# IDEA-Research/MP-Former

Hardware: AMD Instinct MI355X
Metric: training images/sec COCO-instance R50 1024x1024 (higher is better)
Workload: dtype bf16 (backbone, decoder) + f32 (pixel decoder, losses), as the reference's AMP; 1 GPU; COCO-instance R50, 100 queries, 80 classes, 1024x1024: full train step = R50 backbone + MSDeformAttn pixel decoder (6 layers) + MP masked decoder (9 layers, NUM_DN 1) + Hungarian matching + 60 losses + backward + grad all-reduce + clip + AdamW; head_only_workload=False, global_batch=2, per_gpu_batch=2, parallelism=dp1, msda_offsets=init, full=False, autograd_threads=backward on the launch thread, miopen_find_db=shipped

## Files before the change

include/mpformer_hip.h:

```cpp
#ifndef MPFORMER_HIP_H
#define MPFORMER_HIP_H

#include <stddef.h>
#include <stdint.h>

#ifdef __cplusplus
extern "C" {
#endif

enum { MPF_F32 = 0, MPF_F64 = 1, MPF_BF16 = 2, MPF_U8 = 3, MPF_BITS = 4  };

enum {
    MPF_OK = 0,
    MPF_E_DTYPE = -1,
    MPF_E_SHAPE = -2,
    MPF_E_NULL = -3,
    MPF_E_TOO_LARGE = -4
};

int mpf_abi_version(void);
const char* mpf_last_error(void);


int mpf_msda_forward(const void* value, const int64_t* spatial_shapes,
// ... 331 lines not shown
                      int Cout, int transposed, void* stream);
int mpf_gemm3_conv3x3_wgrad(const float* dy, const float* x, float* c_part, float* csum_dy, int n_img, int H, int W, int Cin, int Cout,
                            int rows_per_split, void* stream);

int mpf_gemm3_tn_ex(const void* a, int a_dtype, int64_t lda, const void* b_planes, const float* bias, const float* c_in, int64_t ldcin,
                    void* c, int c_dtype, int64_t ldc, int M, int N, int K, int relu, void* stream);
int mpf_gemm3_nt_ex(const void* a, int a_dtype, int64_t lda, const void* b, int b_dtype, int64_t ldb, float* c_part, float* csum_a,
                    int R, int Mdim, int Ndim, int rows_per_split, void* stream);

typedef struct MpfSplitItem {
    const float* src;
    void* dst;
    int64_t rows, cols, transpose, dst_ld, plane_stride, first_block;
} MpfSplitItem;

int mpf_gemm3_split_grouped(const MpfSplitItem* items_device, int n_items, int64_t total_blocks, void* stream);

typedef struct MpfOptItem {
    float* param;
    const float* grad;
    float* exp_avg;
    float* exp_avg_sq;
    int64_t numel, first_block;
    float lr, weight_decay, bc1, bc2_sqrt;
} MpfOptItem;

int mpf_clip_adamw_step(const MpfOptItem* items_device, int n_items, int64_t total_blocks, float max_norm, double beta1,
                        double beta2, double eps, float* partial, float* norm_clip, void* stream);

int mpf_transpose_f32(const float* in, int64_t in_batch_stride, float* out, int64_t out_batch_stride, int B, int R, int C,
                      void* stream);

int mpf_gemm3_nt_reduce(const float* c_part, int64_t c_numel, const float* s_part, int64_t s_numel, int nsplit,
                        float* c_out, float* s_out, void* stream);
int mpf_gemm3_nt_reduce_levels(const float* c_part, int64_t c_numel, const float* s_part, int64_t s_numel, int nsplit,
                               const int64_t* level_of_split, int n_levels, float* c_out, float* lvl_out, float* s_out, void* stream);

int mpf_tall_gemm_bf16(const void* a, int64_t lda, const void* b, int64_t ldb, const void* bias, void* c, int64_t ldc, int M, int N,
                       int K, void* stream);
size_t mpf_gemm_nt_bf16_workspace_bytes(int R, int Mdim, int Ndim, int rows_per_split);
int mpf_gemm_nt_bf16(const void* a, int64_t lda, const void* b, int64_t ldb, void* c_out, void* csum_out, int R, int Mdim,
                     int Ndim, int rows_per_split, void* workspace, size_t workspace_bytes, void* stream);

int mpf_small_gemm_bf16_blocked(const void* a, int64_t a_rs, int64_t a_ks, int a_blk, int64_t a_bs, const void* gate, const void* b,
                                int64_t b_rs, int64_t b_ks, const void* bias, const void* c_in, int64_t ldcin, void* c, int64_t ldc,
                                int c_blk, int64_t c_bs, void* rowsum_a, int I, int J, int Kc, int relu, void* stream);

int mpf_class_loss_forward(const void* logits, int dtype, int64_t sl, int64_t sn, int64_t sq, const int64_t* target,
                           int target_per_output, const float* weight, int L, int N, int Q, int C, float* lse, float* ce,
                           float* wsum, void* stream);
int mpf_class_loss_backward(const void* logits, int dtype, int64_t sl, int64_t sn, int64_t sq, const int64_t* target,
                            int target_per_output, const float* weight, int L, int N, int Q, int C, const float* lse,
                            const float* wsum, const float* grad_ce, void* dlogits, void* stream);
int mpf_mask_loss_finalize(const float* sums, const int64_t* runs, const float* norm, int n, int G, int points, float* out,
                           void* stream);
int mpf_mask_loss_finalize_backward(const float* sums, const int64_t* runs, const float* norm, int n, int G, int points,
                                    const float* grad_out, float* dsums, void* stream);

typedef struct {
    const void* a;
    const void* gate;
    const void* b;
    void* c;
    void* rowsum_a;
    int64_t a_rs, a_ks, a_bs, b_rs, b_ks, ldc;
    int a_blk, I, J, Kc;
} MpfSmallGemmItem;
int mpf_small_gemm_bf16_group(const MpfSmallGemmItem* items, int n_items, void* stream);
typedef struct MpfTransposeItem {
    const void* src;
    const void* gate;
    void* dst;
    int64_t ld;
    int R, C;
} MpfTransposeItem;
int mpf_transpose_group_bf16(const MpfTransposeItem* items, int n_items, int Rp, void* stream);

int mpf_bias_act(const void* x, const float* bias, const void* res, void* y, int64_t numel, int C, int dtype,
                 int relu, void* stream);
int mpf_relu_bwd_add(const void* ga, const void* gb, const void* y, void* out, int64_t numel, int dtype, void* stream);
int mpf_maxpool3x3s2_forward(const void* x, void* y, void* code, int N, int H, int W, int C, void* stream);
int mpf_maxpool3x3s2_backward(const void* gy, const void* code, void* gx, int N, int H, int W, int C, void* stream);

int mpf_upload_small(const void* host_src, void* device_dst, int64_t nbytes, void* stream);

int mpf_res_ln256_forward(const float* x, const void* t, int t_dtype, const float* gamma, const float* beta,
                          float* s_out, float* y32, void* y16, float* mean, float* rstd, int rows, float eps,
                          const float* padd, int padd_rows, float* y_plus, void* stream);
int mpf_res_ln256_forward_b(const float* x, const void* t, int t_dtype, const float* gamma, const float* beta, float* s_out, float* y32,
                            void* y16, float* mean, float* rstd, int rows, float eps, const float* padd, int padd_rows, float* y_plus,
                            float* y_bound, const float* padd_amax, float* yplus_bound, void* stream);
int mpf_res_ln256_backward(const float* s, const float* mean, const float* rstd, const float* gamma, const float* gy32,
                           const void* gy16, const float* gy_plus, float* ds32, void* ds16, float* dgamma, float* dbeta,
                           int rows, void* stream);
size_t mpf_res_ln256_backward_workspace_bytes(int rows);
int mpf_res_ln256_backward_ws(const float* s, const float* mean, const float* rstd, const float* gamma, const float* gy32,
                              const void* gy16, const float* gy_plus, float* ds32, void* ds16, float* dgamma, float* dbeta, int rows,
                              void* workspace, size_t workspace_bytes, void* stream);
int mpf_res_ln256_backward_ws_amax(const float* s, const float* mean, const float* rstd, const float* gamma, const float* gy32,
                                   const void* gy16, const float* gy_plus, float* ds32, void* ds16, float* dgamma, float* dbeta, int rows,
                                   void* workspace, size_t workspace_bytes, float* ds_amax, void* stream);
int mpf_res_ln256_backward_partial(const float* s, const float* mean, const float* rstd, const float* gamma, const float* gy32,
                                   const void* gy16, const float* gy_plus, float* ds32, void* ds16, int rows, void* partials,
                                   size_t partials_bytes, void* stream);
int mpf_res_ln256_backward_partial_amax(const float* s, const float* mean, const float* rstd, const float* gamma, const float* gy32,
                                        const void* gy16, const float* gy_plus, float* ds32, void* ds16, int rows, void* partials,
                                        size_t partials_bytes, float* ds_amax, void* stream);
int mpf_ln_partial_reduce(const void* partials, size_t stride_bytes, int rows, int n_ln, float* out, void* stream);
size_t mpf_res_ln256_backward_det_workspace_bytes(int rows);
int mpf_res_ln256_backward_det(const float* s, const float* mean, const float* rstd, const float* gamma, const float* gy32,
                               const void* gy16, const float* gy_plus, float* ds32, void* ds16, float* dgamma_dbeta, int rows,
                               void* workspace, size_t workspace_bytes, void* stream);
size_t mpf_res_ln256_backward_workspace_bytes(int rows);
int mpf_res_ln256_backward_ws(const float* s, const float* mean, const float* rstd, const float* gamma, const float* gy32,
                              const void* gy16, const float* gy_plus, float* ds32, void* ds16, float* dgamma, float* dbeta, int rows,
                              void* workspace, size_t workspace_bytes, void* stream);

int mpf_mask_loss_backward_dense(const void* pred, int pred_dtype, int h, int w, const int64_t* pred_rows,
                                 const void* gt, int gt_dtype, int H, int W, const int32_t* gt_rows, const float* coords,
                                 const float* grad_sums, void* grad, int grad_dtype, const int64_t* grad_offs,
                                 int n, int P, void* stream);

size_t mpf_group_stats_workspace_bytes(int rows, int64_t row_len);
int mpf_group_stats(const float* x, int rows, int64_t row_len, float eps, float* mean, float* rstd,
                    void* workspace, size_t workspace_bytes, void* stream);

int mpf_gn_cl_supported(int HW, int C, int G);
size_t mpf_gn_cl_workspace_bytes(int N, int HW, int C, int G);
int mpf_gn_cl_forward(const float* x, int64_t x_bs, const float* gamma, const float* beta, int N, int HW, int C, int G,
                      float eps, int relu, const float* top, int64_t top_bs, int W, float* y, int64_t y_bs, float* mean,
                      float* rstd, void* workspace, size_t workspace_bytes, void* stream);
int mpf_gn_cl_backward(const float* gy, int64_t gy_bs, const float* x, int64_t x_bs, const float* gamma, const float* beta,
                       const float* mean, const float* rstd, int N, int HW, int C, int G, int relu, float* dx,
                       int64_t dx_bs, float* dgamma, float* dbeta, void* workspace, size_t workspace_bytes, void* stream);
int mpf_upsample2x_cl_backward(const float* gy, int64_t gy_bs, int N, int Ht, int Wt, int C, float* dtop, int64_t dtop_bs,
                               void* stream);

size_t mpf_match_cost_fused_workspace_bytes(int G, int Q, int Tmax, int P, int tsamp_rows);
int mpf_match_cost_fused(const void* embed, const int64_t* embed_first, int64_t embed_row_stride, const void* features,
                         int64_t feat_img_stride, const int32_t* group_image, int h, int w, int channels, const float* coords,
                         const float* tsamp, int tsamp_rows, const int32_t* t_first, const int32_t* t_count, float* cost, int G,
                         int Q, int Tmax, int P, float w_mask, float w_dice, void* workspace, size_t workspace_bytes, void* stream);
int mpf_pair_planes_forward(const void* embed, const int64_t* row_off, const int32_t* pair_of_slot, const int32_t* slot_first,
                            const int32_t* slot_count, const void* features, int64_t feat_img_stride, void* out, int N, int HW,
                            int channels, void* stream);
size_t mpf_pair_planes_backward_workspace_bytes(int N, int HW, int total_slots, int max_count);
int mpf_pair_planes_backward(const void* grad_planes, const void* embed, const int64_t* row_off, const int32_t* pair_of_slot,
                             const int32_t* slot_first, const int32_t* slot_count, const void* features, int64_t feat_img_stride,
                             void* d_features, int64_t dfeat_img_stride, void* d_embed, int d_embed_dtype, int N, int HW, int channels,
                             int total_slots, int max_count, void* workspace, size_t workspace_bytes, void* stream);

int mpf_profile_enable(int on);
int mpf_profile_get(const char* name_substr, int* count, double* total_ms, double* total_bytes);
int mpf_profile_get_flops(const char* name_substr, double* total_flops);

enum {
    MPF_ENC_PV, MPF_ENC_PV_AM, MPF_ENC_PO, MPF_ENC_PO_AM, MPF_ENC_P1, MPF_ENC_P1_AM, MPF_ENC_P2, MPF_ENC_P2_AM, MPF_ENC_P288, MPF_ENC_P288_AM,
    MPF_ENC_BV, MPF_ENC_BO, MPF_ENC_BB1, MPF_ENC_BB2, MPF_ENC_B288, MPF_ENC_G1, MPF_ENC_B1, MPF_ENC_G2, MPF_ENC_B2,
    MPF_ENC_VALUE, MPF_ENC_RAW, MPF_ENC_LOC, MPF_ENC_ATTN, MPF_ENC_AO, MPF_ENC_S1, MPF_ENC_MEAN1, MPF_ENC_RSTD1, MPF_ENC_X1, MPF_ENC_H,
    MPF_ENC_HBITS, MPF_ENC_S2, MPF_ENC_MEAN2, MPF_ENC_RSTD2, MPF_ENC_X2, MPF_ENC_QN,
    MPF_ENC_AO_AM, MPF_ENC_X1_AM, MPF_ENC_H_AM, MPF_ENC_XN_AM, MPF_ENC_QN_AM,
    MPF_ENC_FIELDS
};
typedef struct MpfEncoderCall {
    int32_t N, S, M, L, P, nl, F, reserved;
    float eps, pad_;
// ... 117 lines not shown
```

mp_former_amd/_lib.py:

```python
import ctypes

import torch
import os

_HERE = os.path.dirname(os.path.abspath(__file__))
LIB_PATH = os.path.join(_HERE, "libmpformer_hip.so")
LIB_PATH = os.environ.get("MPF_LIB_PATH", LIB_PATH)
ABI_VERSION = 1

MPF_F32, MPF_F64, MPF_BF16, MPF_U8, MPF_BITS = 0, 1, 2, 3, 4
DTYPE = {torch.float32: MPF_F32, torch.float64: MPF_F64, torch.bfloat16: MPF_BF16, torch.uint8: MPF_U8, torch.bool: MPF_U8}

_lib = None
_status_fns = {}

_c_int = ctypes.c_int
_c_vp = ctypes.c_void_p

SIGNATURES = {
    "mpf_abi_version": (_c_int, []),
    "mpf_last_error": (ctypes.c_char_p, []),
    "mpf_last_kernel": (ctypes.c_char_p, []),
    "mpf_set_option": (_c_int, [ctypes.c_char_p, _c_int]),
    "mpf_match_cost_fused_workspace_bytes": (ctypes.c_size_t, [_c_int] * 5),
# ... 34 lines not shown
    "mpf_attn_backward": (_c_int, [_c_vp] * 8 + [_c_int] + [_c_vp] * 5 + [_c_int] * 6 + [ctypes.c_float, _c_vp, ctypes.c_size_t, _c_vp]),
    "mpf_attn_transpose2": (_c_int, [_c_vp] * 4 + [_c_int] * 4 + [_c_vp]),
    "mpf_attn_transpose2_strided": (_c_int, [_c_vp] * 2 + [ctypes.c_int64] * 2 + [_c_vp] * 2 + [_c_int] * 4 + [_c_vp]),
    "mpf_attn_forward_kv": (_c_int, [_c_vp, _c_vp, ctypes.c_int64, ctypes.c_int64, _c_vp, _c_vp, _c_int, _c_vp, _c_vp, _c_int, _c_int,
                                     _c_int, _c_int, _c_int, ctypes.c_float, _c_vp, ctypes.c_size_t, _c_vp]),
    "mpf_attn_backward_kv": (_c_int, [_c_vp] * 3 + [ctypes.c_int64] * 2 + [_c_vp] * 5 + [_c_int] + [_c_vp] * 5 + [ctypes.c_int64] * 2
                             + [_c_int] * 6 + [ctypes.c_float, _c_vp, ctypes.c_size_t, _c_vp]),
    "mpf_attn_backward_kv_aux": (_c_int, [_c_vp] * 3 + [ctypes.c_int64] * 2 + [_c_vp] * 5 + [_c_int] + [_c_vp] * 5 + [ctypes.c_int64] * 2
                                 + [_c_int] * 6 + [ctypes.c_float, _c_vp, ctypes.c_size_t, _c_vp, _c_vp]),
    "mpf_attn_bwd_aux_bytes": (ctypes.c_size_t, [_c_int] * 5),
    "mpf_attn_bwd_prep_aux": (_c_int, [_c_vp] * 5 + [_c_int] * 2 + [_c_vp] * 4 + [ctypes.c_size_t] + [_c_int] * 4 + [_c_vp]),
    "mpf_attn_delta": (_c_int, [_c_vp] * 3 + [_c_int] * 3 + [_c_vp]),
    "mpf_attn_bwd_prep": (_c_int, [_c_vp] * 6 + [_c_int] * 4 + [_c_vp]),
    "mpf_gemm3_split": (_c_int, [_c_vp, _c_int, _c_int, _c_int, _c_vp, _c_vp]),
    "mpf_gemm3_tn": (_c_int, [_c_vp, ctypes.c_int64, _c_vp, _c_int, _c_vp, _c_vp, _c_vp, ctypes.c_int64, _c_vp, ctypes.c_int64,
                           _c_vp, ctypes.c_int64, _c_vp, ctypes.c_int64, _c_int, _c_int, _c_int, _c_int, _c_vp]),
    "mpf_gemm3_nt": (_c_int, [_c_vp, ctypes.c_int64, _c_vp, ctypes.c_int64, _c_vp, ctypes.c_int64, _c_int, _c_vp, _c_vp, _c_vp,
                           _c_int, _c_int, _c_int, _c_int, _c_int, _c_vp]),
    "mpf_amax_f32": (_c_int, [_c_vp, ctypes.c_int64, _c_vp, _c_vp]),
    "mpf_amax_f32_grouped": (_c_int, [_c_vp, _c_int, ctypes.c_int64, _c_vp]),
    "mpf_h2_range_stats": (_c_int, [_c_vp, _c_int, _c_int, ctypes.c_int64, _c_vp, _c_int, _c_vp, _c_vp]),
    "mpf_gemm3_split_grouped_h2": (_c_int, [_c_vp, _c_int, ctypes.c_int64, _c_vp]),
    "mpf_gemm3_tn_h2": (_c_int, [_c_vp, ctypes.c_int64, _c_vp, _c_vp, _c_vp, _c_vp, _c_vp, ctypes.c_int64, _c_vp, ctypes.c_int64,
                              _c_vp, ctypes.c_int64, _c_vp, ctypes.c_int64, _c_vp, _c_int, _c_int, _c_int, _c_int, _c_vp]),
    "mpf_gemm3_tn_h2_bits": (_c_int, [_c_vp, ctypes.c_int64, _c_vp, _c_vp, _c_vp, _c_vp, _c_vp, ctypes.c_int64, _c_vp, ctypes.c_int64,
                                   _c_vp, ctypes.c_int64, _c_vp, ctypes.c_int64, _c_vp, _c_vp, ctypes.c_int64,
                                   _c_int, _c_int, _c_int, _c_int, _c_vp]),
    "mpf_gemm3_nt_h2": (_c_int, [_c_vp, ctypes.c_int64, _c_vp, _c_vp, ctypes.c_int64, _c_vp, _c_vp, _c_vp, _c_vp,
                              _c_int, _c_int, _c_int, _c_int, _c_int, _c_vp]),
    "mpf_gemm3_nt_grouped_h2": (_c_int, [_c_vp, _c_int, _c_int, _c_int, ctypes.c_int64, _c_vp]),
    "mpf_gemm3_conv3x3_h2": (_c_int, [_c_vp] * 7 + [_c_int] * 6 + [_c_vp]),
    "mpf_gemm3_conv3x3_wgrad_h2": (_c_int, [_c_vp, _c_vp, _c_vp, _c_vp, _c_vp, _c_vp, _c_int, _c_int, _c_int, _c_int, _c_int, _c_int, _c_vp]),
    "mpf_gemm3_nt_grouped": (_c_int, [_c_vp, _c_int, _c_int, _c_int, ctypes.c_int64, _c_vp]),
    "mpf_small_gemm_bf16": (_c_int, [_c_vp, ctypes.c_int64, ctypes.c_int64, _c_vp, _c_vp, ctypes.c_int64, ctypes.c_int64, _c_vp, _c_vp,
                                     ctypes.c_int64, _c_vp, ctypes.c_int64, _c_vp, _c_int, _c_int, _c_int, _c_int, _c_vp]),
    "mpf_encoder_fields": (_c_int, []),
    "mpf_encoder_forward": (_c_int, [_c_vp, _c_vp]),
    "mpf_encoder_bwd_fields": (_c_int, []),
    "mpf_encoder_backward": (_c_int, [_c_vp, _c_vp]),
    "mpf_decoder_layer_struct_bytes": (ctypes.c_uint64, [_c_int]),
    "mpf_decoder_layer_scratch_bytes": (ctypes.c_uint64, [_c_int] * 6),
    "mpf_decoder_layer_forward": (_c_int, [_c_vp, _c_vp]),
    "mpf_next_attn_mask_scratch_bytes": (ctypes.c_size_t, [_c_int, _c_int]),
    "mpf_next_attn_mask": (_c_int, [_c_vp, _c_vp]),
    "mpf_lin256_res_ln_forward": (_c_int, [_c_vp] * 11 + [_c_int, ctypes.c_float, _c_vp]),
    "mpf_ln256_mlp3_forward": (_c_int, [_c_vp] * 10 + [_c_int, ctypes.c_float, _c_vp]),
    "mpf_decoder_layer_backward": (_c_int, [_c_vp, _c_vp, _c_vp]),
    "mpf_pool_features": (_c_int, [_c_vp, _c_int, _c_vp] + [_c_int] * 6 + [_c_vp]),
    "mpf_pool_features_cl": (_c_int, [_c_vp, ctypes.c_int64, _c_int, _c_vp, _c_int, _c_int, _c_int, _c_int, _c_int, _c_int, _c_vp]),
    "mpf_mask_head_bits": (_c_int, [_c_vp, ctypes.c_int64, ctypes.c_int64, _c_vp, _c_vp, _c_int, _c_vp, _c_vp] + [_c_int] * 3 + [_c_vp]),
    "mpf_lsa_assign": (_c_int, [_c_vp, _c_vp, _c_int, _c_int, ctypes.c_int64] + [_c_vp] * 7),
    "mpf_lsa_assign_status": (_c_int, [_c_vp, _c_vp, _c_int, _c_int, ctypes.c_int64] + [_c_vp] * 8),
    "mpf_mask_block_empty": (_c_int, [_c_vp, _c_vp] + [_c_int] * 5 + [_c_vp]),
    "mpf_mp_open_counts": (_c_int, [_c_vp, _c_int, _c_int, _c_vp, _c_vp]),
    "mpf_mp_noise_rows": (_c_int, [_c_vp] * 3 + [_c_int] * 4 + [ctypes.c_double, ctypes.c_uint64, ctypes.c_uint64, _c_vp, _c_vp]),
    "mpf_gemm_nt_bf16_workspace_bytes": (ctypes.c_size_t, [_c_int] * 4),
    "mpf_gemm_nt_bf16": (_c_int, [_c_vp, ctypes.c_int64, _c_vp, ctypes.c_int64, _c_vp, _c_vp, _c_int, _c_int, _c_int, _c_int, _c_vp,
                                  ctypes.c_size_t, _c_vp]),
    "mpf_gemm3_nt_reduce": (_c_int, [_c_vp, ctypes.c_int64, _c_vp, ctypes.c_int64, _c_int, _c_vp, _c_vp, _c_vp]),
    "mpf_grouped_scale_cast": (_c_int, [_c_vp, _c_int, ctypes.c_int64, _c_int, _c_int, _c_vp]),
    "mpf_gemm3_split_grouped": (_c_int, [_c_vp, _c_int, ctypes.c_int64, _c_vp]),
    "mpf_decoder_inputs_forward": (_c_int, [_c_vp, ctypes.c_int64, ctypes.c_int64, _c_vp, _c_vp, _c_vp, _c_vp, _c_int, _c_int, _c_int, _c_int,
                                            _c_vp]),
    "mpf_decoder_inputs_backward": (_c_int, [_c_vp, _c_vp, _c_int, _c_vp, ctypes.c_int64, ctypes.c_int64, _c_int, _c_int, _c_int, _c_vp]),
    "mpf_clip_inputs_forward": (_c_int, [_c_vp, ctypes.c_int64, ctypes.c_int64, _c_vp, _c_vp, _c_vp, _c_vp, _c_vp, _c_int, _c_int, _c_int, _c_int,
                                         _c_int, _c_vp]),
    "mpf_clip_inputs_backward": (_c_int, [_c_vp, _c_vp, _c_int, _c_vp, ctypes.c_int64, ctypes.c_int64, _c_int, _c_int, _c_int, _c_int, _c_vp]),
    "mpf_clip_adamw_step": (_c_int, [_c_vp, _c_int, ctypes.c_int64, ctypes.c_float, ctypes.c_double, ctypes.c_double, ctypes.c_double,
                                     _c_vp, _c_vp, _c_vp]),
    "mpf_transpose_f32": (_c_int, [_c_vp, ctypes.c_int64, _c_vp, ctypes.c_int64, _c_int, _c_int, _c_int, _c_vp]),
    "mpf_small_gemm_bf16_blocked": (_c_int, [_c_vp, ctypes.c_int64, ctypes.c_int64, _c_int, ctypes.c_int64, _c_vp, _c_vp, ctypes.c_int64,
                                             ctypes.c_int64, _c_vp, _c_vp, ctypes.c_int64, _c_vp, ctypes.c_int64, _c_int, ctypes.c_int64,
                                             _c_vp, _c_int, _c_int, _c_int, _c_int, _c_vp]),
    "mpf_small_gemm_bf16_group": (_c_int, [_c_vp, _c_int, _c_vp]),
    "mpf_transpose_group_bf16": (_c_int, [_c_vp, _c_int, _c_int, _c_vp]),
    "mpf_class_loss_forward": (_c_int, [_c_vp, _c_int, ctypes.c_int64, ctypes.c_int64, ctypes.c_int64, _c_vp, _c_int, _c_vp, _c_int, _c_int,
                                        _c_int, _c_int, _c_vp, _c_vp, _c_vp, _c_vp]),
    "mpf_class_loss_backward": (_c_int, [_c_vp, _c_int, ctypes.c_int64, ctypes.c_int64, ctypes.c_int64, _c_vp, _c_int, _c_vp, _c_int, _c_int,
                                         _c_int, _c_int, _c_vp, _c_vp, _c_vp, _c_vp, _c_vp]),
    "mpf_mask_loss_finalize": (_c_int, [_c_vp, _c_vp, _c_vp, _c_int, _c_int, _c_int, _c_vp, _c_vp]),
    "mpf_mask_loss_finalize_backward": (_c_int, [_c_vp, _c_vp, _c_vp, _c_int, _c_int, _c_int, _c_vp, _c_vp, _c_vp]),
    "mpf_bias_act": (_c_int, [_c_vp, _c_vp, _c_vp, _c_vp, ctypes.c_int64, _c_int, _c_int, _c_int, _c_vp]),
    "mpf_relu_bwd_add": (_c_int, [_c_vp, _c_vp, _c_vp, _c_vp, ctypes.c_int64, _c_int, _c_vp]),
    "mpf_maxpool3x3s2_forward": (_c_int, [_c_vp] * 3 + [_c_int] * 4 + [_c_vp]),
    "mpf_maxpool3x3s2_backward": (_c_int, [_c_vp] * 3 + [_c_int] * 4 + [_c_vp]),
    "mpf_upload_small": (_c_int, [_c_vp, _c_vp, ctypes.c_int64, _c_vp]),
    "mpf_tall_gemm_bf16": (_c_int, [_c_vp, ctypes.c_int64, _c_vp, ctypes.c_int64, _c_vp, _c_vp, ctypes.c_int64, _c_int, _c_int, _c_int, _c_vp]),
    "mpf_res_ln256_forward": (_c_int, [_c_vp, _c_vp, _c_int, _c_vp, _c_vp, _c_vp, _c_vp, _c_vp, _c_vp, _c_vp, _c_int, ctypes.c_float,
                                       _c_vp, _c_int, _c_vp, _c_vp]),
    "mpf_res_ln256_forward_b": (_c_int, [_c_vp, _c_vp, _c_int, _c_vp, _c_vp, _c_vp, _c_vp, _c_vp, _c_vp, _c_vp, _c_int, ctypes.c_float,
                                         _c_vp, _c_int, _c_vp, _c_vp, _c_vp, _c_vp, _c_vp]),
    "mpf_res_ln256_backward_ws_amax": (_c_int, [_c_vp] * 11 + [_c_int, _c_vp, ctypes.c_size_t, _c_vp, _c_vp]),
    "mpf_res_ln256_backward": (_c_int, [_c_vp] * 11 + [_c_int, _c_vp]),
    "mpf_mask_loss_backward_dense": (_c_int, [_c_vp, _c_int, _c_int, _c_int, _c_vp, _c_vp, _c_int, _c_int, _c_int, _c_vp, _c_vp, _c_vp,
                                              _c_vp, _c_int, _c_vp, _c_int, _c_int, _c_vp]),
    "mpf_gn_cl_supported": (_c_int, [_c_int, _c_int, _c_int]),
    "mpf_gn_cl_workspace_bytes": (ctypes.c_size_t, [_c_int, _c_int, _c_int, _c_int]),
    "mpf_gn_cl_forward": (_c_int, [_c_vp, ctypes.c_int64, _c_vp, _c_vp, _c_int, _c_int, _c_int, _c_int, ctypes.c_float, _c_int,
                                   _c_vp, ctypes.c_int64, _c_int, _c_vp, ctypes.c_int64, _c_vp, _c_vp, _c_vp, ctypes.c_size_t, _c_vp]),
    "mpf_gn_cl_backward": (_c_int, [_c_vp, ctypes.c_int64, _c_vp, ctypes.c_int64, _c_vp, _c_vp, _c_vp, _c_vp, _c_int, _c_int, _c_int,
                                    _c_int, _c_int, _c_vp, ctypes.c_int64, _c_vp, _c_vp, _c_vp, ctypes.c_size_t, _c_vp]),
    "mpf_upsample2x_cl_backward": (_c_int, [_c_vp, ctypes.c_int64, _c_int, _c_int, _c_int, _c_int, _c_vp, ctypes.c_int64, _c_vp]),
    "mpf_gemm3_conv3x3": (_c_int, [_c_vp, _c_vp, _c_vp, _c_vp, _c_int, _c_int, _c_int, _c_int, _c_int, _c_int, _c_vp]),
    "mpf_gemm3_conv3x3_wgrad": (_c_int, [_c_vp, _c_vp, _c_vp, _c_vp, _c_int, _c_int, _c_int, _c_int, _c_int, _c_int, _c_vp]),
    "mpf_gemm3_nt_reduce_levels": (_c_int, [_c_vp, ctypes.c_int64, _c_vp, ctypes.c_int64, _c_int, _c_vp, _c_int, _c_vp, _c_vp, _c_vp, _c_vp]),
    "mpf_gemm3_tn_ex": (_c_int, [_c_vp, _c_int, ctypes.c_int64, _c_vp, _c_vp, _c_vp, ctypes.c_int64, _c_vp, _c_int, ctypes.c_int64,
                                 _c_int, _c_int, _c_int, _c_int, _c_vp]),
    "mpf_gemm3_nt_ex": (_c_int, [_c_vp, _c_int, ctypes.c_int64, _c_vp, _c_int, ctypes.c_int64, _c_vp, _c_vp, _c_int, _c_int, _c_int, _c_int, _c_vp]),
    "mpf_res_ln256_backward_workspace_bytes": (ctypes.c_size_t, [_c_int]),
    "mpf_res_ln256_backward_partial": (_c_int, [_c_vp] * 9 + [_c_int, _c_vp, ctypes.c_size_t, _c_vp]),
    "mpf_res_ln256_backward_partial_amax": (_c_int, [_c_vp] * 9 + [_c_int, _c_vp, ctypes.c_size_t, _c_vp, _c_vp]),
    "mpf_ln_partial_reduce": (_c_int, [_c_vp, ctypes.c_size_t, _c_int, _c_int, _c_vp, _c_vp]),
    "mpf_res_ln256_backward_det_workspace_bytes": (ctypes.c_size_t, [_c_int]),
    "mpf_res_ln256_backward_det": (_c_int, [_c_vp] * 10 + [_c_int, _c_vp, ctypes.c_size_t, _c_vp]),
    "mpf_res_ln256_backward_ws": (_c_int, [_c_vp] * 11 + [_c_int, _c_vp, ctypes.c_size_t, _c_vp]),
    "mpf_group_stats_workspace_bytes": (ctypes.c_size_t, [_c_int, ctypes.c_int64]),
    "mpf_group_stats": (_c_int, [_c_vp, _c_int, ctypes.c_int64, ctypes.c_float, _c_vp, _c_vp, _c_vp, ctypes.c_size_t, _c_vp]),
    "mpf_msda_forward": (_c_int, [_c_vp] * 6 + [_c_int] * 8 + [_c_vp]),
    "mpf_msda_backward": (_c_int, [_c_vp] * 9 + [_c_int] * 8 + [_c_vp]),
    "mpf_msda_forward_hs": (_c_int, [_c_vp] * 7 + [_c_int] * 8 + [_c_vp]),
    "mpf_msda_forward_raw_hs": (_c_int, [_c_vp] * 9 + [_c_int] * 8 + [_c_vp]),
    "mpf_msda_forward_raw": (_c_int, [_c_vp] * 8 + [_c_int] * 8 + [_c_vp]),
    "mpf_msda_backward_ws_raw": (_c_int, [_c_vp] * 7 + [_c_int] * 8 + [_c_vp, ctypes.c_size_t, _c_vp]),
    "mpf_msda_backward_ws_raw_o": (_c_int, [_c_vp] * 8 + [_c_int] * 8 + [_c_vp, ctypes.c_size_t, _c_vp, _c_vp, _c_vp]),
    "mpf_msda_backward_workspace_bytes": (ctypes.c_size_t, [_c_int] * 5 + [_c_vp]),
    "mpf_msda_backward_ws": (_c_int, [_c_vp] * 8 + [_c_int] * 8 + [_c_vp, ctypes.c_size_t, _c_vp]),
    "mpf_seg_softmax": (_c_int, [_c_vp, _c_int, _c_int, ctypes.c_float] + [_c_vp] * 6),
    "mpf_seg_semantic": (_c_int, [_c_vp, ctypes.c_int64] + [_c_int] * 10 + [_c_vp, _c_int, _c_vp, _c_vp]),
    "mpf_seg_instance_workspace_bytes": (ctypes.c_size_t, [_c_int] * 3),
    "mpf_seg_instance_scores": (_c_int, [_c_vp, ctypes.c_int64] + [_c_int] * 10 + [_c_vp, _c_vp, _c_int, _c_vp, _c_vp, ctypes.c_size_t,
                                                                                   _c_vp]),
    "mpf_seg_instance_masks": (_c_int, [_c_vp, ctypes.c_int64] + [_c_int] * 10 + [_c_vp, _c_int, _c_vp, _c_vp]),
    "mpf_seg_panoptic_areas": (_c_int, [_c_vp, ctypes.c_int64] + [_c_int] * 10 + [_c_vp] * 5),
    "mpf_seg_panoptic_paint": (_c_int, [_c_vp, _c_int, _c_int, _c_vp, _c_vp, _c_vp]),
    "mpf_seg_semantic_labels": (_c_int, [_c_vp, ctypes.c_int64] + [_c_int] * 10 + [_c_vp, _c_int, _c_vp, _c_vp]),
    "mpf_seg_labels_resize": (_c_int, [_c_vp] + [_c_int] * 5 + [_c_vp, _c_vp]),
    "mpf_seg_confusion_add": (_c_int, [_c_vp, _c_vp, ctypes.c_int64, _c_int, _c_int, _c_vp, _c_vp]),
    "mpf_seg_instance_rle_workspace_bytes": (ctypes.c_size_t, [_c_int] * 3),
    "mpf_seg_instance_rle_count": (_c_int, [_c_vp, ctypes.c_int64] + [_c_int] * 10 + [_c_vp, _c_int, _c_vp, _c_vp, ctypes.c_size_t, _c_vp]),
    "mpf_seg_instance_rle_write": (_c_int, [_c_vp, ctypes.c_size_t, _c_int, _c_int, _c_int, _c_vp, ctypes.c_int64, _c_vp, _c_vp, _c_vp]),
    "mpf_seg_tta_accumulate": (_c_int, [_c_vp, ctypes.c_int64] + [_c_int] * 10 + [_c_vp, _c_int, _c_int, _c_vp, _c_vp]),
    "mpf_seg_tta_resize_add": (_c_int, [_c_vp] + [_c_int] * 6 + [_c_vp, _c_vp]),
    "mpf_seg_tta_finish": (_c_int, [_c_vp] + [_c_int] * 4 + [_c_vp, _c_vp]),
    "mpf_seg_pq_workspace_bytes": (ctypes.c_size_t, [_c_int] * 2),
    "mpf_seg_pq_pairs": (_c_int, [_c_vp, _c_vp, _c_int, ctypes.c_int64, _c_vp, _c_int, _c_int, _c_vp, _c_int, _c_int, _c_int, _c_vp,
                                  ctypes.c_size_t, _c_vp]),
    "mpf_seg_pq_match": (_c_int, [_c_vp, ctypes.c_size_t, _c_int, _c_int, _c_int, _c_vp, _c_vp, _c_vp, _c_int] + [_c_vp] * 6),
    "mpf_seg_instance_bits": (_c_int, [_c_vp, ctypes.c_int64] + [_c_int] * 10 + [_c_vp, _c_int, _c_vp, _c_vp]),
    "mpf_seg_pack_masks": (_c_int, [_c_vp, _c_int, _c_int, _c_int, _c_int, _c_vp, _c_vp]),
    "mpf_seg_mask_pairs": (_c_int, [_c_vp, _c_int, _c_vp, _c_int, ctypes.c_int64, _c_vp, _c_vp, _c_vp, _c_vp]),
    "mpf_seg_ap_workspace_bytes": (ctypes.c_size_t, [_c_int] * 3),
    "mpf_seg_ap_match": (_c_int, [_c_vp, _c_vp, _c_vp, _c_int, _c_int] + [_c_vp] * 6 + [_c_int, _c_vp] + [_c_int] * 5
                         + [_c_vp, _c_vp, _c_vp, ctypes.c_size_t, _c_vp]),
    "mpf_seg_mask_boundary": (_c_int, [_c_vp, _c_int, _c_int, _c_int, _c_int, _c_vp, _c_vp]),
    "mpf_seg_ap_match_boundary": (_c_int, [_c_vp] * 6 + [_c_int, _c_int] + [_c_vp] * 6 + [_c_int, _c_vp] + [_c_int] * 5
                                  + [_c_vp, _c_vp, _c_vp, ctypes.c_size_t, _c_vp]),
    "mpf_seg_video_bits": (_c_int, [_c_vp, ctypes.c_int64, ctypes.c_int64] + [_c_int] * 11 + [_c_vp, _c_int, _c_vp, _c_vp, _c_vp, _c_vp]),
    "mpf_seg_tube_areas": (_c_int, [_c_vp, _c_int, _c_int, _c_vp, _c_vp]),
    "mpf_seg_ap_match_tube": (_c_int, [_c_vp, _c_vp, _c_vp, _c_int, _c_int] + [_c_vp] * 7 + [_c_int, _c_vp] + [_c_int] * 5
                              + [_c_vp, _c_vp, _c_vp, ctypes.c_size_t, _c_vp]),
    "mpf_seg_bits_rle_workspace_bytes": (ctypes.c_size_t, [_c_int] * 3),
    "mpf_seg_bits_rle_count": (_c_int, [_c_vp, _c_int, _c_int, _c_int, _c_vp, _c_vp, ctypes.c_size_t, _c_vp]),
    "mpf_seg_bits_rle_write": (_c_int, [_c_vp, _c_vp, ctypes.c_size_t, _c_int, _c_int, _c_int, _c_vp, ctypes.c_int64, _c_vp, _c_vp, _c_vp]),
}


class NativeLibraryError(RuntimeError):
    pass


def lib():
    global _lib
    if _lib is None:
        if not os.path.exists(LIB_PATH):
            raise NativeLibraryError(
                f"{LIB_PATH} not found: build it with `python -c 'import __graft_entry__ as g; g.build()'` "
                "or `make -C mp_former_amd/csrc`.  mp_former_amd has no CPU / eager fallback.")
        l = ctypes.CDLL(LIB_PATH)
        for name, (res, args) in SIGNATURES.items():
            try:
                fn = getattr(l, name)
            except AttributeError as e:
                raise NativeLibraryError(f"{LIB_PATH} does not export {name}") from e
            fn.restype = res
            fn.argtypes = args
            if res is _c_int:
                _status_fns[name] = fn
        v = l.mpf_abi_version()
        if v != ABI_VERSION:
            raise NativeLibraryError(f"ABI mismatch: library {v}, binding {ABI_VERSION}")
        _lib = l
        for kv in filter(None, os.environ.get("MPF_OPTIONS", "").split(",")):
            k, _, v = kv.partition("=")
            set_option(k.strip(), int(v))
    return _lib


def check(code, what):
    if code != 0:
        msg = lib().mpf_last_error().decode()
        raise RuntimeError(f"{what} failed with code {code}: {msg}")


def _status_fn(name):
    lib()
    fn = _status_fns.get(name)
    if fn is None:
        raise TypeError(f"{name} does not return a status: call() is for the int-returning entry points, sizes go through lib()")
    return fn


def call(name, device, *args):
    fn = _status_fns.get(name) or _status_fn(name)
    idx = device.index
    if idx is None or idx == torch.cuda.current_device():
        code = fn(*args)
    else:
        with torch.cuda.device(device):
            code = fn(*args)
    if code != 0:
        check(code, name)


def ptr(t):
    return None if t is None else t.data_ptr()


_option_gen = 0


def option_generation():
    return _option_gen


def set_option(key, value):
    global _option_gen
    check(lib().mpf_set_option(key.encode(), int(value)), f"mpf_set_option({key})")
    _option_gen += 1


def msda_stats(reset=True):
    out = (ctypes.c_ulonglong * 9)()
    check(lib().mpf_msda_stats(out, 9, 1 if reset else 0), "mpf_msda_stats")
    keys = ("fwd_lds", "fwd_gather", "push_lds", "push_gather", "push_direct", "push_hash", "spill_entries", "pull_split", "pull_single")
    return dict(zip(keys, (int(v) for v in out)))


def last_kernel():
    return lib().mpf_last_kernel().decode()


def profile_enable(on=True):
    check(lib().mpf_profile_enable(1 if on else 0), "mpf_profile_enable")


def profile_get_flops(name_substr):
    fl = ctypes.c_double(0)
    check(lib().mpf_profile_get_flops(name_substr.encode(), ctypes.byref(fl)), "mpf_profile_get_flops")
    return fl.value


def profile_get(name_substr):
    n, ms, by = _c_int(0), ctypes.c_double(0), ctypes.c_double(0)
    check(lib().mpf_profile_get(name_substr.encode(), ctypes.byref(n), ctypes.byref(ms), ctypes.byref(by)),
          "mpf_profile_get")
    return n.value, ms.value, by.value


_scratch = {}


def scratch(owner, device, stream, nbytes, zeroed=False):
    key = (owner, device, stream)
    w = _scratch.get(key)
    if w is None or w.numel() < nbytes:
        n = int(nbytes * 1.25) + 1024
        w = _scratch[key] = (torch.zeros if zeroed else torch.empty)(n, dtype=torch.uint8, device=device)
    return w


def stream_ptr(device):
    idx = device.index
    return torch._C._cuda_getCurrentRawStream(torch.cuda.current_device() if idx is None else idx)


class _NullGuard:
    def __enter__(self):
        return None

    def __exit__(self, *exc):
        return False


_NULL_GUARD = _NullGuard()


def device_guard(device):
    idx = device.index
    if idx is None or idx == torch.cuda.current_device():
        return _NULL_GUARD
    return torch.cuda.device(device)
```

mp_former_amd/backbone.py:

```python
import numpy as np
import torch
import torch.nn.functional as F
from torch import nn

from . import _lib
from ._h2d import upload


class FrozenBatchNorm2d(nn.Module):

    def __init__(self, num_features, eps=1e-5):
        super().__init__()
        self.eps = eps
        self.register_buffer("weight", torch.ones(num_features))
        self.register_buffer("bias", torch.zeros(num_features))
        self.register_buffer("running_mean", torch.zeros(num_features))
        self.register_buffer("running_var", torch.ones(num_features))

    def scale_bias(self):
        b = self._buffers
        w, bb, rm, rv = b["weight"], b["bias"], b["running_mean"], b["running_var"]
        c = self.__dict__.get("_sb_cache")
        if (c is None or c[0] is not w or c[1] is not bb or c[2] is not rm or c[3] is not rv
                or c[4] != (w._version, bb._version, rm._version, rv._version)):
            with torch.no_grad():
                scale = w * (rv + self.eps).rsqrt()
                c = (w, bb, rm, rv, (w._version, bb._version, rm._version, rv._version), scale,
                     (bb - rm * scale).float().contiguous())
            self.__dict__["_sb_cache"] = c
        return c[5], c[6]

    def forward(self, x):
        scale, bias = self.scale_bias()
        return x * scale.to(x.dtype).view(1, -1, 1, 1) + bias.to(x.dtype).view(1, -1, 1, 1)


class _BiasAct(torch.autograd.Function):

    @staticmethod
    def forward(ctx, x, shift, res, relu):
        y = torch.empty_like(x)
        C = x.shape[1]
        _lib.call("mpf_bias_act", x.device, x.data_ptr(), shift.data_ptr(), _lib.ptr(res), y.data_ptr(), x.numel(), C,
                  _lib.DTYPE[x.dtype], 1 if relu else 0, _lib.stream_ptr(x.device))
        ctx.relu, ctx.has_res = relu, res is not None
        if relu:
            ctx.save_for_backward(y)
        return y

    @staticmethod
    def backward(ctx, g):
        if ctx.relu:
            (y,) = ctx.saved_tensors
            g = torch.ops.aten.threshold_backward(g, y, 0)
        return g, None, (g if ctx.has_res else None), None


def _relu_bwd_add(ga, gb, y):
    same = (ga.dtype == torch.bfloat16 and y.dtype == torch.bfloat16 and ga.shape == y.shape and ga.stride() == y.stride() and _dense(y)
            and ga.numel() % 8 == 0 and (gb is None or (gb.dtype == ga.dtype and gb.shape == ga.shape and gb.stride() == ga.stride())))
    if not (ga.is_cuda and same):
        return torch.ops.aten.threshold_backward(ga if gb is None else ga + gb, y, 0)
    out = torch.empty_like(y)
    _lib.call("mpf_relu_bwd_add", y.device, ga.data_ptr(), _lib.ptr(gb), y.data_ptr(), out.data_ptr(), y.numel(), _lib.MPF_BF16,
              _lib.stream_ptr(y.device))
    return out


class _BiasActFork(torch.autograd.Function):

    @staticmethod
    def forward(ctx, x, shift, res):
        y = torch.empty_like(x)
        _lib.call("mpf_bias_act", x.device, x.data_ptr(), shift.data_ptr(), res.data_ptr(), y.data_ptr(), x.numel(), x.shape[1],
                  _lib.DTYPE[x.dtype], 1, _lib.stream_ptr(x.device))
        ctx.save_for_backward(y)
        ctx.set_materialize_grads(False)
        return y, y.view(y.shape)

    @staticmethod
    def backward(ctx, ga, gb):
        (y,) = ctx.saved_tensors
        if ga is None and gb is None:
            return None, None, None
        if ga is None:
            ga, gb = gb, None
        g = _relu_bwd_add(ga, gb, y)
        return g, None, g


def _bias_act_ok(x, res):
    return (x.is_cuda and x.dim() == 4 and x.dtype in (torch.bfloat16, torch.float32) and x.shape[1] % 8 == 0
            and x.is_contiguous(memory_format=torch.channels_last)
            and (res is None or (res.dtype == x.dtype and res.shape == x.shape
                                 and res.is_contiguous(memory_format=torch.channels_last))))


def bias_act(x, shift, res=None, relu=True):
    if _bias_act_ok(x, res):
        return _BiasAct.apply(x, shift, res, relu)
    y = x + shift.to(x.dtype).view(1, -1, 1, 1)
    if res is not None:
        y = y + res
    return F.relu(y) if relu else y


def bias_act_fork(x, shift, res):
    if _bias_act_ok(x, res) and x.dtype == torch.bfloat16:
        return _BiasActFork.apply(x, shift, res)
    y = bias_act(x, shift, res, True)
    return y, y


class _MaxPool3x3s2(torch.autograd.Function):

    @staticmethod
    def forward(ctx, x):
        N, C, H, W = x.shape
        OH, OW = (H - 1) // 2 + 1, (W - 1) // 2 + 1
        y = torch.empty((N, C, OH, OW), dtype=x.dtype, device=x.device, memory_format=torch.channels_last)
        code = torch.empty((N, OH, OW, C), dtype=torch.uint8, device=x.device)
        _lib.call("mpf_maxpool3x3s2_forward", x.device, x.data_ptr(), y.data_ptr(), code.data_ptr(), N, H, W, C,
                  _lib.stream_ptr(x.device))
        ctx.save_for_backward(code)
        ctx.in_shape = (N, C, H, W)
        return y

    @staticmethod
    def backward(ctx, gy):
        (code,) = ctx.saved_tensors
        N, C, H, W = ctx.in_shape
        if gy.dtype != torch.bfloat16 or not gy.is_contiguous(memory_format=torch.channels_last):
            gy = gy.to(torch.bfloat16).contiguous(memory_format=torch.channels_last)
        gx = torch.empty((N, C, H, W), dtype=gy.dtype, device=gy.device, memory_format=torch.channels_last)
        _lib.call("mpf_maxpool3x3s2_backward", gy.device, gy.data_ptr(), code.data_ptr(), gx.data_ptr(), N, H, W, C,
                  _lib.stream_ptr(gy.device))
        return gx


def max_pool_3x3_s2(x):
    if (x.is_cuda and x.dim() == 4 and x.dtype == torch.bfloat16 and x.shape[1] % 8 == 0 and 256 % (x.shape[1] // 8) == 0
            and x.is_contiguous(memory_format=torch.channels_last)):
        return _MaxPool3x3s2.apply(x)
    return F.max_pool2d(x, kernel_size=3, stride=2, padding=1)


def conv_bn(conv, bn, x, folded=None, res=None, relu=True, fork=False):
    if folded is not None:
        w, shift = folded
    else:
        scale, shift = bn.scale_bias()
        w = conv.weight * scale.view(-1, 1, 1, 1)
    y = F.conv2d(x, w, None, conv.stride, conv.padding, conv.dilation, conv.groups)
    return bias_act_fork(y, shift, res) if fork else bias_act(y, shift, res, relu)


def _dense(t):
    return t.is_contiguous() or (t.dim() == 4 and t.is_contiguous(memory_format=torch.channels_last))


_gsc_layouts = {}


def _grouped_scale_cast(srcs, scales, out_dtype):
    dev = srcs[0].device
    key = tuple([(t.shape, t.stride()) for t in srcs] + [id(sc) for sc in scales] + [out_dtype])
    lay = _gsc_layouts.get(key)
    if lay is None:
        numels = [t.numel() for t in srcs]
        offs, tot, blk = [], 0, 0
        table = np.zeros((len(srcs), 6), dtype=np.int64)
        for i, (t, sc) in enumerate(zip(srcs, scales)):
            assert _dense(t) and sc.dtype == torch.float32 and sc.is_contiguous() and sc.numel() == t.shape[0]
            offs.append(tot)
            table[i, 2:] = (sc.data_ptr(), numels[i], numels[i] // t.shape[0], blk)
            tot += (numels[i] + 63) & ~63
            blk += (numels[i] + 2047) // 2048
        esz = torch.empty(0, dtype=out_dtype).element_size()
        lay = (table, np.asarray(offs, dtype=np.int64) * esz, tot, blk, [(o, n, t.shape, t.stride()) for o, n, t in zip(offs, numels, srcs)],
               list(scales))
        if len(_gsc_layouts) > 64:
            _gsc_layouts.clear()
        _gsc_layouts[key] = lay
    table, offs_b, tot, blk, views, _ = lay
    out = torch.empty(tot, dtype=out_dtype, device=dev)
    table[:, 0] = [t.data_ptr() for t in srcs]
    table[:, 1] = offs_b + out.data_ptr()
    items = upload(table.reshape(-1), dev)
    _lib.call("mpf_grouped_scale_cast", dev, items.data_ptr(), len(srcs), blk, _lib.DTYPE[srcs[0].dtype], _lib.DTYPE[out_dtype],
              _lib.stream_ptr(dev))
    return [out[o:o + n].as_strided(shp, std) for o, n, shp, std in views]


class _FoldCast(torch.autograd.Function):

    @staticmethod
    def forward(ctx, dtype, scales, *weights):
        ctx.scales = scales
        ws = [p.detach() for p in weights]
        native = (ws[0].is_cuda and all(w.dtype == torch.float32 and _dense(w) for w in ws)
                  and dtype in (None, torch.float32, torch.bfloat16))
        ctx.native = native
        if native:
            return tuple(_grouped_scale_cast(ws, scales, dtype or torch.float32))
        w = torch._foreach_mul(ws, [s_.view(-1, 1, 1, 1) for s_ in scales])
        if dtype is None:
            return tuple(w)
        outs = [torch.empty_like(t, dtype=dtype) for t in w]
        torch._foreach_copy_(outs, w)
        return tuple(outs)

    @staticmethod
    def backward(ctx, *grads):
        if ctx.native and all(g is not None and g.dtype == grads[0].dtype for g in grads) \
                and grads[0].dtype in (torch.float32, torch.bfloat16):
            gs = [g if _dense(g) else g.contiguous() for g in grads]
            return (None, None, *_grouped_scale_cast(gs, ctx.scales, torch.float32))
        g32 = [torch.empty_like(g, dtype=torch.float32) for g in grads]
        torch._foreach_copy_(g32, list(grads))
        torch._foreach_mul_(g32, [s_.view(-1, 1, 1, 1) for s_ in ctx.scales])
        return (None, None, *g32)


_PAIR_NAMES = (("conv1", "norm1"), ("conv2", "norm2"), ("conv3", "norm3"), ("shortcut", "shortcut_norm"))


class Bottleneck(nn.Module):
    def __init__(self, cin, cmid, cout, stride):
        super().__init__()
        self.shortcut = None
        if cin != cout or stride != 1:
            self.shortcut = nn.Conv2d(cin, cout, 1, stride=stride, bias=False)
            self.shortcut_norm = FrozenBatchNorm2d(cout)
        self.conv1 = nn.Conv2d(cin, cmid, 1, bias=False)
        self.norm1 = FrozenBatchNorm2d(cmid)
        self.conv2 = nn.Conv2d(cmid, cmid, 3, stride=stride, padding=1, bias=False)
        self.norm2 = FrozenBatchNorm2d(cmid)
        self.conv3 = nn.Conv2d(cmid, cout, 1, bias=False)
        self.norm3 = FrozenBatchNorm2d(cout)

    def pairs(self):
        m = self._modules
        p = self.__dict__.get("_pairs")
        if p is not None:
            names = _PAIR_NAMES if len(p) == 4 else _PAIR_NAMES[:3]
            if (m.get("shortcut") is None) != (len(p) == 3) or any(c is not m.get(cn) or n is not m.get(nn_) for (c, n), (cn, nn_) in zip(p, names)):
                p = None
        if p is None:
            p = [(self.conv1, self.norm1), (self.conv2, self.norm2), (self.conv3, self.norm3)]
            if self.shortcut is not None:
                p.append((self.shortcut, self.shortcut_norm))
            self.__dict__["_pairs"] = p
        return p

    def forward(self, x, fw=None):
        return self.forward_fork((x, x), fw)[0]

    def forward_fork(self, xs, fw=None):
        f = fw if fw is not None else [None] * 4
        x_main, x_skip = xs
        p = self.pairs()
        out = conv_bn(p[0][0], p[0][1], x_main, f[0])
        out = conv_bn(p[1][0], p[1][1], out, f[1])
        sc = x_skip if len(p) == 3 else conv_bn(p[3][0], p[3][1], x_skip, f[3], relu=False)
        return conv_bn(p[2][0], p[2][1], out, f[2], res=sc, fork=True)


class ResNet50(nn.Module):
    def __init__(self):
        super().__init__()
        self.stem_conv = nn.Conv2d(3, 64, 7, stride=2, padding=3, bias=False)
        self.stem_norm = FrozenBatchNorm2d(64)
        cfg = [("res2", 3, 64, 256, 1), ("res3", 4, 128, 512, 2), ("res4", 6, 256, 1024, 2), ("res5", 3, 512, 2048, 2)]
        cin = 64
        self.stage_names = []
        for name, n, cmid, cout, stride in cfg:
            blocks = []
            for i in range(n):
                blocks.append(Bottleneck(cin, cmid, cout, stride if i == 0 else 1))
                cin = cout
            setattr(self, name, nn.Sequential(*blocks))
            self.stage_names.append(name)
        for m in self.modules():
            if isinstance(m, nn.Conv2d):
                nn.init.kaiming_normal_(m.weight, mode="fan_out", nonlinearity="relu")

    @staticmethod
    def _fold_group(pairs, dtype):
        sb = [bn.scale_bias() for _, bn in pairs]
        scales = [s_ for s_, _ in sb]
        ws = _FoldCast.apply(dtype, scales, *[c.weight for c, _ in pairs])
        return [(w, b_) for w, (_, b_) in zip(ws, sb)]

    def forward(self, x):
        return self.forward_stages(x, self.stage_names, stem=True)

    def forward_stages(self, x, names, stem=False):
        return run_stages(x, [(n, getattr(self, n)) for n in names], (self.stem_conv, self.stem_norm) if stem else None)


def run_stages(x, stages, stem=None):
    dtype = torch.get_autocast_dtype("cuda") if (torch.is_autocast_enabled() and x.is_cuda) else None
    if stem is not None:
        st = ResNet50._fold_group([stem], dtype)
        x = conv_bn(stem[0], stem[1], x, st[0])
        x = max_pool_3x3_s2(x)
    out = {}
    for name, stage in stages:
        blocks = list(stage)
        folded = ResNet50._fold_group([p for b in blocks for p in b.pairs()], dtype)
        k = 0
        xs = x if isinstance(x, tuple) else (x, x)
        for b in blocks:
            n = len(b.pairs())
            xs = b.forward_fork(xs, folded[k:k + n])
            k += n
        x = xs
        out[name] = xs[0]
    return out
```

mp_former_amd/csrc/elementwise.hip:

```cpp
#include <hip/hip_bf16.h>
#include <hip/hip_runtime.h>
#include <stdint.h>

#include "mpf_common.h"
#include "amax.h"

namespace {

typedef __attribute__((ext_vector_type(8))) __bf16 bf16x8;

template <bool RES>
__global__ __launch_bounds__(256) void bias_act_bf16_kernel(const bf16x8* __restrict__ x, const float* __restrict__ bias,
                                                            const bf16x8* __restrict__ res, bf16x8* __restrict__ y,
                                                            int64_t n8, int C, int relu)
{
    for (int64_t i = (int64_t)blockIdx.x * blockDim.x + threadIdx.x; i < n8; i += (int64_t)gridDim.x * blockDim.x) {
        const bf16x8 v = x[i];
        const int c0 = (int)((i * 8) % C);
        const float4 b0 = *reinterpret_cast<const float4*>(bias + c0);
        const float4 b1 = *reinterpret_cast<const float4*>(bias + c0 + 4);
        const float b[8] = {b0.x, b0.y, b0.z, b0.w, b1.x, b1.y, b1.z, b1.w};
        bf16x8 r = {0, 0, 0, 0, 0, 0, 0, 0};
        if constexpr (RES) r = res[i];
        bf16x8 o;
// ... 643 lines not shown
    }
    mean[row] = (float)mu;
    rstd[row] = (float)(1.0 / sqrt(m2 / n + (double)eps));
}

}

extern "C" size_t mpf_group_stats_workspace_bytes(int rows, int64_t row_len)
{
    if (rows <= 0 || row_len <= 0) return 0;
    const int64_t chunks = (row_len + kGnThreads * kGnPer - 1) / (kGnThreads * kGnPer);
    return (size_t)rows * chunks * 3 * sizeof(float);
}

extern "C" int mpf_group_stats(const float* x, int rows, int64_t row_len, float eps, float* mean, float* rstd,
                               void* workspace, size_t workspace_bytes, void* stream)
{
    hipStream_t st = (hipStream_t)stream;
    if (!x || !mean || !rstd || !workspace) return mpf::fail(MPF_E_NULL, "group_stats: NULL buffer");
    if (rows <= 0 || row_len <= 0 || row_len % 4 != 0) return mpf::fail(MPF_E_SHAPE, "group_stats: row length must be a positive multiple of 4");
    if (workspace_bytes < mpf_group_stats_workspace_bytes(rows, row_len)) return mpf::fail(MPF_E_SHAPE, "group_stats: workspace too small");
    const int chunks = (int)((row_len + kGnThreads * kGnPer - 1) / (kGnThreads * kGnPer));
    mpf::prof_begin(st);
    mpf::set_kernel("gn_chunk_stats_kernel");
    hipLaunchKernelGGL(gn_chunk_stats_kernel, dim3(chunks, rows), dim3(kGnThreads), 0, st, x, (float*)workspace, row_len, chunks);
    mpf::prof_end(mpf_last_kernel(), st, 4.0 * (double)rows * (double)row_len);
    hipLaunchKernelGGL(gn_merge_kernel, dim3((rows + 63) / 64), dim3(64), 0, st, (const float*)workspace, mean, rstd, rows, chunks, eps);
    return mpf::check(hipGetLastError(), "mpf_group_stats");
}

namespace {

constexpr int kGsPer = 8;
constexpr int kGsBlock = 256 * kGsPer;

template <typename TS, typename TD>
__global__ __launch_bounds__(256) void grouped_scale_cast_kernel(const MpfScaleCastItem* __restrict__ items, int n_items)
{
    int lo = 0, hi = n_items - 1;
    const int64_t blk = blockIdx.x;
    while (lo < hi) {
        const int mid = (lo + hi + 1) >> 1;
        if (items[mid].first_block <= blk) lo = mid; else hi = mid - 1;
    }
    const MpfScaleCastItem it = items[lo];
    const TS* __restrict__ src = static_cast<const TS*>(it.src);
    TD* __restrict__ dst = static_cast<TD*>(it.dst);
    const float* __restrict__ scale = it.scale;
    const int64_t base = (blk - it.first_block) * kGsBlock;
#pragma unroll
    for (int k = 0; k < kGsPer; ++k) {
        const int64_t e = base + (int64_t)k * 256 + threadIdx.x;
        if (e < it.numel) {
            const float v = (float)src[e] * scale[e / it.inner];
            dst[e] = (TD)v;
        }
    }
}

}

extern "C" int mpf_grouped_scale_cast(const MpfScaleCastItem* items_device, int n_items, int64_t total_blocks, int src_dtype,
                                      int dst_dtype, void* stream)
{
    if (n_items == 0 || total_blocks == 0) return 0;
    if (!items_device) return mpf::fail(MPF_E_NULL, "grouped_scale_cast: NULL table");
    if (n_items < 0 || total_blocks < 0 || total_blocks > 0x7fffffffLL) return mpf::fail(MPF_E_SHAPE, "grouped_scale_cast: bad sizes");
    hipStream_t st = (hipStream_t)stream;
    const dim3 grid((unsigned)total_blocks);
    mpf::set_kernel("grouped_scale_cast_kernel");
    if (src_dtype == MPF_F32 && dst_dtype == MPF_BF16)
        hipLaunchKernelGGL((grouped_scale_cast_kernel<float, __bf16>), grid, dim3(256), 0, st, items_device, n_items);
    else if (src_dtype == MPF_BF16 && dst_dtype == MPF_F32)
        hipLaunchKernelGGL((grouped_scale_cast_kernel<__bf16, float>), grid, dim3(256), 0, st, items_device, n_items);
    else if (src_dtype == MPF_F32 && dst_dtype == MPF_F32)
        hipLaunchKernelGGL((grouped_scale_cast_kernel<float, float>), grid, dim3(256), 0, st, items_device, n_items);
    else
        return mpf::fail(MPF_E_DTYPE, "grouped_scale_cast: (src, dst) must be (f32, bf16), (bf16, f32) or (f32, f32)");
    return mpf::check(hipGetLastError(), "mpf_grouped_scale_cast");
}

namespace {

constexpr int kOptBlock = 2048;

__device__ __forceinline__ const MpfOptItem& opt_item_of(const MpfOptItem* __restrict__ items, int n_items, int64_t blk)
{
    int lo = 0, hi = n_items - 1;
    while (lo < hi) {
        const int mid = (lo + hi + 1) >> 1;
        if (items[mid].first_block <= blk) lo = mid; else hi = mid - 1;
    }
    return items[lo];
}

__global__ __launch_bounds__(256) void opt_sqnorm_kernel(const MpfOptItem* __restrict__ items, int n_items, float* __restrict__ partial)
{
    __shared__ float red[4];
    const MpfOptItem& it = opt_item_of(items, n_items, blockIdx.x);
    const float* __restrict__ g = it.grad;
    const int64_t base = ((int64_t)blockIdx.x - it.first_block) * kOptBlock;
    float s = 0.f;
#pragma unroll
    for (int k = 0; k < kOptBlock / 256; ++k) {
        const int64_t e = base + (int64_t)k * 256 + threadIdx.x;
        const float v = e < it.numel ? g[e] : 0.f;
        s += v * v;
    }
    s = wave_sum(s);
    if ((threadIdx.x & 63) == 0) red[threadIdx.x >> 6] = s;
    __syncthreads();
    if (threadIdx.x == 0) partial[blockIdx.x] = (red[0] + red[1]) + (red[2] + red[3]);
}

__global__ __launch_bounds__(1024) void opt_clip_coef_kernel(const float* __restrict__ partial, int64_t n, float max_norm, float* __restrict__ out)
{
    __shared__ double red[16];
    double s = 0.0;
    for (int64_t i = threadIdx.x; i < n; i += 1024) s += (double)partial[i];
#pragma unroll
    for (int o = 32; o > 0; o >>= 1) s += __shfl_xor(s, o);
    if ((threadIdx.x & 63) == 0) red[threadIdx.x >> 6] = s;
    __syncthreads();
    if (threadIdx.x == 0) {
        double t = 0.0;
        for (int w = 0; w < 16; ++w) t += red[w];
        const float norm = (float)sqrt(t);
        out[0] = norm;
        out[1] = max_norm > 0.f ? fminf(max_norm / (norm + 1e-6f), 1.0f) : 1.0f;
    }
}

__global__ __launch_bounds__(256) void opt_adamw_kernel(const MpfOptItem* __restrict__ items, int n_items, const float* __restrict__ clip,
                                                        float one_minus_beta1, float beta2, float one_minus_beta2, float eps)
{
    const MpfOptItem& it = opt_item_of(items, n_items, blockIdx.x);
    float* __restrict__ p = it.param;
    const float* __restrict__ g = it.grad;
    float* __restrict__ m = it.exp_avg;
    float* __restrict__ v = it.exp_avg_sq;
    const float c = clip ? clip[1] : 1.0f;
    const float decay = 1.0f - it.lr * it.weight_decay, step_size = it.lr / it.bc1, bc2_sqrt = it.bc2_sqrt;
    const int64_t base = ((int64_t)blockIdx.x - it.first_block) * kOptBlock;
#pragma unroll
    for (int k = 0; k < kOptBlock / 256; ++k) {
        const int64_t e = base + (int64_t)k * 256 + threadIdx.x;
        if (e < it.numel) {
            const float gr = g[e] * c;
            float pe = p[e] * decay;
            const float me = m[e] + (gr - m[e]) * one_minus_beta1;
            const float ve = beta2 * v[e] + one_minus_beta2 * gr * gr;
            const float denom = sqrtf(ve) / bc2_sqrt + eps;
            pe -= step_size * (me / denom);
            p[e] = pe; m[e] = me; v[e] = ve;
        }
    }
}

}

extern "C" int mpf_clip_adamw_step(const MpfOptItem* items_device, int n_items, int64_t total_blocks, float max_norm, double beta1,
                                   double beta2, double eps, float* partial, float* norm_clip, void* stream)
{
    if (n_items == 0 || total_blocks == 0) return 0;
    if (!items_device || !partial || !norm_clip) return mpf::fail(MPF_E_NULL, "clip_adamw_step: NULL buffer");
    if (n_items < 0 || total_blocks < 0 || total_blocks > 0x7fffffffLL) return mpf::fail(MPF_E_SHAPE, "clip_adamw_step: bad sizes");
// ... 64 lines not shown
```

mp_former_amd/csrc/gemm3.hip:

```cpp
#include <hip/hip_runtime.h>

#include <algorithm>
#include <atomic>
#include <stdint.h>
#include <stdio.h>

#include "mpf_common.h"
#include "amax.h"
#ifndef G3_PRIO
#define G3_PRIO 1
#endif

namespace {

typedef __attribute__((ext_vector_type(8))) __bf16 bf16x8;
typedef __attribute__((ext_vector_type(4))) float f32x4;

constexpr int kBM = 128;
constexpr int kBK = 32;
constexpr int kThreads = 256;
constexpr int kAKc = kBM * 16;

struct G3 {
    const float* a;
    const float* a2;
    const unsigned short* bp;
    const float* bias;
    const float* cin;
    const float* cin2;
    const float* gate;
    float* c;
    int64_t lda, ldc, ldcin, ldcin2, ldgate, plane;
    int M, N, K, a2_rows, relu, tiles_n, ntiles;
    int bias_cm, cin_cm, cin2_cm, gate_cm;
    unsigned short* c16;
    int cv_H, cv_W, cv_cin, cv_sign;
    int tm0, ntiles2, tiles_n2;
    const float* a_amax;
    const float* b_amax;
    float* out_amax;
    const unsigned char* gbits;
    unsigned char* gbits_out;
    int64_t ldgbits, ldgbits_out;
    int gbits_cm;
    int t3_bm;
};

int g_ablate = 0;
int g_mixed = 1;
int g_two_pass = 256;
int g_two_pass_rows = 0;
int g_nt2 = 1;
int g_tn3 = 1;
int g_tn3_176 = 1;
int g_ws = 512;


__device__ __forceinline__ unsigned pack_hi16(unsigned a, unsigned b)
{
    return __builtin_amdgcn_perm(b, a, 0x07060302u);
}

__device__ __forceinline__ void split8(const float4 u, const float4 v, uint4* h, uint4* m, uint4* l)
{
    const float x[8] = {u.x, u.y, u.z, u.w, v.x, v.y, v.z, v.w};
    unsigned hb[8], mb[8], lb[8];
#pragma unroll
    for (int i = 0; i < 8; ++i) {
        const unsigned xb = __float_as_uint(x[i]);
        hb[i] = xb;
        const float r1 = x[i] - __uint_as_float(xb & 0xFFFF0000u);
        const unsigned rb = __float_as_uint(r1);
        mb[i] = rb;
        const float r2 = r1 - __uint_as_float(rb & 0xFFFF0000u);
        lb[i] = __float_as_uint(r2) + 0x8000u;
    }
    *h = make_uint4(pack_hi16(hb[0], hb[1]), pack_hi16(hb[2], hb[3]), pack_hi16(hb[4], hb[5]), pack_hi16(hb[6], hb[7]));
    *m = make_uint4(pack_hi16(mb[0], mb[1]), pack_hi16(mb[2], mb[3]), pack_hi16(mb[4], mb[5]), pack_hi16(mb[6], mb[7]));
    *l = make_uint4(pack_hi16(lb[0], lb[1]), pack_hi16(lb[2], lb[3]), pack_hi16(lb[4], lb[5]), pack_hi16(lb[6], lb[7]));
}

typedef __attribute__((ext_vector_type(8))) _Float16 f16x8;
typedef __attribute__((ext_vector_type(2))) _Float16 f16x2;
typedef __attribute__((ext_vector_type(2))) float f32x2;

__device__ __forceinline__ void split8h(const float4 u, const float4 v, const float scale, uint4* h, uint4* l)
{
    const float x[8] = {u.x, u.y, u.z, u.w, v.x, v.y, v.z, v.w};
    unsigned hb[4], lb[4];
#pragma unroll
    for (int i = 0; i < 4; ++i) {
        const f32x2 s = {x[2 * i] * scale, x[2 * i + 1] * scale};
        const f16x2 hh = __builtin_convertvector(s, f16x2);
        const f32x2 back = __builtin_convertvector(hh, f32x2);
        const f32x2 r = {s[0] - back[0], s[1] - back[1]};
        const f16x2 ll = __builtin_convertvector(r, f16x2);
        union { f16x2 f; unsigned u; } ch, cl;
        ch.f = hh; cl.f = ll;
        hb[i] = ch.u; lb[i] = cl.u;
    }
    *h = make_uint4(hb[0], hb[1], hb[2], hb[3]);
    *l = make_uint4(lb[0], lb[1], lb[2], lb[3]);
}

__device__ __forceinline__ void h2_scale(const unsigned amax_bits, float* scale, float* inv)
{
    int e = (int)((amax_bits >> 23) & 0xffu);
    e = max(e, 30);
    *scale = __uint_as_float((unsigned)(268 - e) << 23);
    *inv = __uint_as_float((unsigned)(e - 14) << 23);
}

__device__ __forceinline__ f16x8 as_fragh(const uint4 v)
{
    union { uint4 u; f16x8 f; } c;
    c.u = v;
    return c.f;
}

__device__ __forceinline__ float4 add4(float4 x, float4 y) { return make_float4(x.x + y.x, x.y + y.y, x.z + y.z, x.w + y.w); }

__device__ __forceinline__ bf16x8 as_frag(const uint4 v)
{
    union { uint4 u; bf16x8 f; } c;
    c.u = v;
    return c.f;
}

typedef __attribute__((ext_vector_type(16))) float f32x16;

template <int NJ, bool W32 = false>
struct Acc {
    f32x4 v[4][NJ];

    __device__ __forceinline__ void zero()
    {
#pragma unroll
        for (int i = 0; i < 4; ++i)
// ... 118 lines not shown
            for (int j = 0; j < 2; ++j)
#pragma unroll
                for (int e = 0; e < 16; ++e) v[i][j][e] = 0.f;
    }

    template <int AKC, int BKC, bool ONE = false, bool A1 = false, bool B1 = false>
    __device__ __forceinline__ void step(const unsigned char* lds, int a_base, int b_base, int lane)
    {
        const int r32 = lane & 31, gh = lane >> 5;
#pragma unroll
        for (int kh = 0; kh < 2; ++kh) {
            const int kc = 2 * kh + gh;
            const int sw = (r32 ^ (2 * kc)) * 16;
            if (ONE) {
                bf16x8 fa0[2], fb0[2];
#pragma unroll
                for (int t = 0; t < 2; ++t) {
                    fa0[t] = as_frag(*reinterpret_cast<const uint4*>(lds + a_base + kc * AKC + t * 512 + sw));
                    fb0[t] = as_frag(*reinterpret_cast<const uint4*>(lds + b_base + kc * BKC + t * 512 + sw));
                }
#pragma unroll
                for (int j = 0; j < 2; ++j)
#pragma unroll
                    for (int i = 0; i < 2; ++i) v[i][j] = __builtin_amdgcn_mfma_f32_32x32x16_bf16(fb0[j], fa0[i], v[i][j], 0, 0, 0);
                continue;
            }
            bf16x8 fa[3][2], fb[3][2];
#pragma unroll
            for (int pl = 0; pl < 3; ++pl)
#pragma unroll
                for (int t = 0; t < 2; ++t) {
                    if (pl == 0 || !A1) fa[pl][t] = as_frag(*reinterpret_cast<const uint4*>(lds + a_base + (pl * 4 + kc) * AKC + t * 512 + sw));
                    if (pl == 0 || !B1) fb[pl][t] = as_frag(*reinterpret_cast<const uint4*>(lds + b_base + (pl * 4 + kc) * BKC + t * 512 + sw));
                }
#define G3_MMA32(PB, PA)                                                                                          \
    if ((PA == 0 || !A1) && (PB == 0 || !B1)) {                                                                   \
        _Pragma("unroll") for (int j = 0; j < 2; ++j) _Pragma("unroll") for (int i = 0; i < 2; ++i)               \
            v[i][j] = __builtin_amdgcn_mfma_f32_32x32x16_bf16(fb[PB][j], fa[PA][i], v[i][j], 0, 0, 0);            \
    }
            G3_MMA32(0, 2) G3_MMA32(2, 0) G3_MMA32(1, 1) G3_MMA32(0, 1) G3_MMA32(1, 0) G3_MMA32(0, 0)
#undef G3_MMA32
        }
    }

    template <int AKC, int BKC>
    __device__ __forceinline__ void step_h2(const unsigned char* lds, int a_base, int b_base, int lane)
    {
        const int r32 = lane & 31, gh = lane >> 5;
#pragma unroll
        for (int kh = 0; kh < 2; ++kh) {
            const int kc = 2 * kh + gh;
            const int sw = (r32 ^ (2 * kc)) * 16;
            f16x8 fa[2][2], fb[2][2];
#pragma unroll
            for (int pl = 0; pl < 2; ++pl)
#pragma unroll
                for (int t = 0; t < 2; ++t) {
                    fa[pl][t] = as_fragh(*reinterpret_cast<const uint4*>(lds + a_base + (pl * 4 + kc) * AKC + t * 512 + sw));
                    fb[pl][t] = as_fragh(*reinterpret_cast<const uint4*>(lds + b_base + (pl * 4 + kc) * BKC + t * 512 + sw));
                }
#define G3_MMA32H(PB, PA)                                                                                         \
    _Pragma("unroll") for (int j = 0; j < 2; ++j) _Pragma("unroll") for (int i = 0; i < 2; ++i)                   \
        v[i][j] = __builtin_amdgcn_mfma_f32_32x32x16_f16(fb[PB][j], fa[PA][i], v[i][j], 0, 0, 0);
            G3_MMA32H(1, 0) G3_MMA32H(0, 1) G3_MMA32H(0, 0)
#undef G3_MMA32H
        }
    }

    template <typename F>
    __device__ __forceinline__ void quads(int lane, F f) const
    {
        const int r32 = lane & 31, gh = lane >> 5;
#pragma unroll
        for (int j = 0; j < 2; ++j)
#pragma unroll
            for (int i = 0; i < 2; ++i)
#pragma unroll
                for (int q = 0; q < 4; ++q)
                    f(i * 32 + r32, j * 32 + 8 * q + 4 * gh,
                      make_float4(v[i][j][4 * q], v[i][j][4 * q + 1], v[i][j][4 * q + 2], v[i][j][4 * q + 3]));
    }
};

__device__ __attribute__((aligned(16))) unsigned g3_const[12] = {0u, 0u, 0u, 0u, 0x3f800000u, 0x3f800000u, 0x3f800000u, 0x3f800000u,
                                    0xffffffffu, 0xffffffffu, 0xffffffffu, 0xffffffffu};

int g3_consts(const float** out, const char* who)
{
    constexpr int kMaxDev = mpf::kMaxDevices;
    static std::atomic<const float*> cache[kMaxDev];
    int dev = 0;
    if (hipError_t e = hipGetDevice(&dev); e != hipSuccess) return mpf::check(e, who);
    const float* c = (dev >= 0 && dev < kMaxDev) ? cache[dev].load(std::memory_order_acquire) : nullptr;
    if (!c) {
        void* sym = nullptr;
        if (hipError_t e = hipGetSymbolAddress(&sym, HIP_SYMBOL(g3_const)); e != hipSuccess) return mpf::check(e, who);
        c = (const float*)sym;
        if (dev >= 0 && dev < kMaxDev) cache[dev].store(c, std::memory_order_release);
    }
    *out = c;
    return 0;
}

template <int NJ, int NI = 4, typename AccT = Acc<NJ, false>, bool SCALED = false, bool PIPE = false>
__device__ __forceinline__ float g3_epilogue(const G3& p, const AccT& acc, int lane, int m_wave, int n_wave, const float inv_a = 1.f,
                                            const float inv_b = 1.f, const int m_end = 0x7fffffff)
{
    float amax = 0.f;
    const int r16 = lane & 15, g = lane >> 4;
    int64_t mrow[NI];
    bool mok[NI];
    uint2 gb[NI];
    unsigned wb[NI][2];
#pragma unroll
    for (int i = 0; i < NI; ++i) {
        const int m = m_wave + i * 16 + r16;
        mok[i] = m < p.M && m < m_end;
        mrow[i] = min(m, p.M - 1);
        if constexpr (NJ <= 2) {
            gb[i].x = *reinterpret_cast<const unsigned*>(p.gbits + mrow[i] * p.ldgbits + (n_wave >> 3) * p.gbits_cm);
            gb[i].y = 0u;
        } else {
            gb[i] = *reinterpret_cast<const uint2*>(p.gbits + mrow[i] * p.ldgbits + (n_wave >> 3) * p.gbits_cm);
        }
        wb[i][0] = wb[i][1] = 0u;
    }
    struct Ops { float4 bz, ci[NI], c2[NI], gt[NI]; };
    auto load_ops = [&](const int j, Ops& q) {
        const int nc = min(n_wave + j * 16 + g * 4, p.N - 4);
        q.bz = *reinterpret_cast<const float4*>(p.bias + nc * p.bias_cm);
#pragma unroll
        for (int i = 0; i < NI; ++i) {
            q.ci[i] = *reinterpret_cast<const float4*>(p.cin + mrow[i] * p.ldcin + nc * p.cin_cm);
            q.c2[i] = *reinterpret_cast<const float4*>(p.cin2 + mrow[i] * p.ldcin2 + nc * p.cin2_cm);
            q.gt[i] = *reinterpret_cast<const float4*>(p.gate + mrow[i] * p.ldgate + nc * p.gate_cm);
        }
    };
    Ops ops[2];
    if constexpr (PIPE) load_ops(0, ops[0]);
#pragma unroll
    for (int j = 0; j < NJ; ++j) {
        const int n = n_wave + j * 16 + g * 4;
        const bool nok = n < p.N;
        if constexpr (PIPE) {
            if (j + 1 < NJ) load_ops(j + 1, ops[(j + 1) & 1]);
            __builtin_amdgcn_sched_barrier(0);
        } else {
            load_ops(j, ops[j & 1]);
        }
        const float4 bz = ops[j & 1].bz;
        const float4(&ci)[NI] = ops[j & 1].ci;
        const float4(&c2)[NI] = ops[j & 1].c2;
        const float4(&gt)[NI] = ops[j & 1].gt;
#pragma unroll
        for (int i = 0; i < NI; ++i) {
            float4 o = make_float4(acc.v[i][j][0], acc.v[i][j][1], acc.v[i][j][2], acc.v[i][j][3]);
            if constexpr (SCALED)
                o = make_float4(o.x * inv_a * inv_b, o.y * inv_a * inv_b, o.z * inv_a * inv_b, o.w * inv_a * inv_b);
            o = make_float4(o.x + bz.x, o.y + bz.y, o.z + bz.z, o.w + bz.w);
            o = make_float4(o.x + ci[i].x, o.y + ci[i].y, o.z + ci[i].z, o.w + ci[i].w);
            o = make_float4(o.x + c2[i].x, o.y + c2[i].y, o.z + c2[i].z, o.w + c2[i].w);
            if (p.relu) o = make_float4(fmaxf(o.x, 0.f), fmaxf(o.y, 0.f), fmaxf(o.z, 0.f), fmaxf(o.w, 0.f));
            o = make_float4(gt[i].x > 0.f ? o.x : 0.f, gt[i].y > 0.f ? o.y : 0.f, gt[i].z > 0.f ? o.z : 0.f, gt[i].w > 0.f ? o.w : 0.f);
            if (p.gbits_cm) {
                const unsigned nib = ((j & 2) ? gb[i].y : gb[i].x) >> ((j & 1) * 16 + g * 4);
                o = make_float4((nib & 1u) ? o.x : 0.f, (nib & 2u) ? o.y : 0.f, (nib & 4u) ? o.z : 0.f, (nib & 8u) ? o.w : 0.f);
            }
            if (p.gbits_out) {
                const unsigned pos = (o.x > 0.f ? 1u : 0u) | (o.y > 0.f ? 2u : 0u) | (o.z > 0.f ? 4u : 0u) | (o.w > 0.f ? 8u : 0u);
                wb[i][(j >> 1) & 1] |= pos << ((j & 1) * 16 + g * 4);
            }
            if (mok[i] && nok) {
                if constexpr (SCALED) amax = fmaxf(fmaxf(amax, fmaxf(fabsf(o.x), fabsf(o.y))), fmaxf(fabsf(o.z), fabsf(o.w)));
                if (p.c16) {
                    unsigned w[4];
                    const float e[4] = {o.x, o.y, o.z, o.w};
#pragma unroll
                    for (int t = 0; t < 4; ++t) {
                        unsigned u = __float_as_uint(e[t]);
                        u += 0x7fffu + ((u >> 16) & 1u);
                        w[t] = u >> 16;
                    }
                    *reinterpret_cast<uint2*>(p.c16 + mrow[i] * p.ldc + n) = make_uint2(w[0] | (w[1] << 16), w[2] | (w[3] << 16));
                } else {
                    *reinterpret_cast<float4*>(p.c + mrow[i] * p.ldc + n) = o;
                }
            }
        }
    }
    if (p.gbits_out) {
#pragma unroll
        for (int i = 0; i < NI; ++i) {
            unsigned lo = wb[i][0], hi = wb[i][1];
            lo |= __shfl_xor(lo, 16); hi |= __shfl_xor(hi, 16);
            lo |= __shfl_xor(lo, 32); hi |= __shfl_xor(hi, 32);
            if (g == 0 && mok[i] && n_wave < p.N) {
                if constexpr (NJ <= 2) *reinterpret_cast<unsigned*>(p.gbits_out + mrow[i] * p.ldgbits_out + (n_wave >> 3)) = lo;
                else *reinterpret_cast<uint2*>(p.gbits_out + mrow[i] * p.ldgbits_out + (n_wave >> 3)) = make_uint2(lo, hi);
            }
        }
    }
    return amax;
}

__device__ __forceinline__ void glds16(const void* base, unsigned voff, unsigned lds_addr)
{
    unsigned saved;
    asm volatile("s_mov_b32 %0, m0\n\ts_mov_b32 m0, %3\n\ts_nop 0\n\tglobal_load_lds_dwordx4 %1, %2\n\ts_mov_b32 m0, %0"
                 : "=&s"(saved) : "v"(voff), "s"(base), "s"(lds_addr) : "memory");
}

#include "gemm3_ws.h"
#include "gemm3_tn3.h"

template <int BN, bool A2, bool CV = false, bool ABF = false, bool H2 = false>
__device__ __forceinline__ void g3_tn_tile(const G3& p, unsigned char* lds, const int m0, const int n0)
{
    static_assert(!(ABF && (A2 || CV)), "bf16 A: no addend, no convolution mode");
    static_assert(!(H2 && (ABF || A2)), "fp16 x 2 form: fp32 A, no addend rows");
    constexpr int NJ = BN / 32;
    constexpr int kBKc = BN * 16;
    constexpr int kPl = H2 ? 2 : 3;
    constexpr int kAbytes = kPl * 4 * kAKc;
    constexpr int kBunits = 3 * BN * 4;
    constexpr int kBiter = (kBunits + kThreads - 1) / kThreads;
    constexpr int kBstage = kPl * 4 * kBKc;
    constexpr int kPieces = kBstage / 1024;
    constexpr int kPW = (kPieces + 3) / 4;

    const int tid = threadIdx.x, lane = tid & 63, wave = tid >> 6;
    const int wr = wave >> 1, wc = wave & 1;


    const int akc = tid & 3;
    const int arow0 = tid >> 2, arow1 = 64 + (tid >> 2);
    const int aslot0 = arow0 ^ (2 * akc), aslot1 = arow1 ^ (2 * akc);
    const float* ap0 = ABF ? reinterpret_cast<const float*>(reinterpret_cast<const unsigned short*>(p.a) +
                                                              (int64_t)min(m0 + arow0, p.M - 1) * p.lda + akc * 8)
                           : p.a + (int64_t)min(m0 + arow0, p.M - 1) * p.lda + akc * 8;
    const float* ap1 = ABF ? reinterpret_cast<const float*>(reinterpret_cast<const unsigned short*>(p.a) +
                                                              (int64_t)min(m0 + arow1, p.M - 1) * p.lda + akc * 8)
                           : p.a + (int64_t)min(m0 + arow1, p.M - 1) * p.lda + akc * 8;
    const float* a2p0 = nullptr;
    const float* a2p1 = nullptr;
    if (p.a2) {
        a2p0 = p.a2 + (int64_t)(min(m0 + arow0, p.M - 1) % p.a2_rows) * p.K + akc * 8;
        a2p1 = p.a2 + (int64_t)(min(m0 + arow1, p.M - 1) % p.a2_rows) * p.K + akc * 8;
    }
    int cy0 = 0, cx0 = 0, cy1 = 0, cx1 = 0, mr0 = 0, mr1 = 0;
    if constexpr (CV) {
        mr0 = min(m0 + arow0, p.M - 1); mr1 = min(m0 + arow1, p.M - 1);
        cx0 = mr0 % p.cv_W; cy0 = (mr0 / p.cv_W) % p.cv_H;
        cx1 = mr1 % p.cv_W; cy1 = (mr1 / p.cv_W) % p.cv_H;
    }
    (void)ap0; (void)ap1;
    unsigned boff[kPW];
    int bpiece[kPW];
    {
        const int nl = lane >> 2, kc = (lane & 3) ^ ((0 - (nl >> 2)) & 3);
#pragma unroll
        for (int i = 0; i < kPW; ++i) {
            const int q = min(wave + 4 * i, kPieces - 1);
            const int pl = q / (BN / 16), nb = (q % (BN / 16)) * 16;
            boff[i] = (unsigned)(((int64_t)pl * p.plane + (int64_t)min(n0 + nb + nl, p.N - 1) * p.K + kc * 8) * 2);
            bpiece[i] = __builtin_amdgcn_readfirstlane(q * 1024);
        }
    }
    const unsigned lds_b = (unsigned)(uintptr_t)(lds + kAbytes);

    float4 raE[4], raO[4], ra2[4];
    (void)kBunits; (void)kBiter;
#define G3_LOAD_A(ra, k0)                                                                    \
    {                                                                                        \
        ra[0] = *reinterpret_cast<const float4*>(ap0 + (k0));                                \
        ra[1] = *reinterpret_cast<const float4*>(ap0 + (k0) + 4);                            \
        ra[2] = *reinterpret_cast<const float4*>(ap1 + (k0));                                \
        ra[3] = *reinterpret_cast<const float4*>(ap1 + (k0) + 4);                            \
    }
#define G3_LOAD_A_CV(ra, vm, k0)                                                             \
    {                                                                                        \
        const int tap_ = (k0) / p.cv_cin, kk_ = (k0) - tap_ * p.cv_cin;                      \
        const int dy_ = (tap_ / 3 - 1) * p.cv_sign, dx_ = (tap_ % 3 - 1) * p.cv_sign;        \
        const int sh_ = dy_ * p.cv_W + dx_;                                                  \
        const bool v0_ = (unsigned)(cy0 + dy_) < (unsigned)p.cv_H && (unsigned)(cx0 + dx_) < (unsigned)p.cv_W; \
        const bool v1_ = (unsigned)(cy1 + dy_) < (unsigned)p.cv_H && (unsigned)(cx1 + dx_) < (unsigned)p.cv_W; \
         \
        const unsigned o0_ = (unsigned)(min(max(mr0 + sh_, 0), p.M - 1) * (int)p.lda + akc * 8 + kk_); \
        const unsigned o1_ = (unsigned)(min(max(mr1 + sh_, 0), p.M - 1) * (int)p.lda + akc * 8 + kk_); \
        ra[0] = *reinterpret_cast<const float4*>(p.a + o0_);                                 \
        ra[1] = *reinterpret_cast<const float4*>(p.a + o0_ + 4);                             \
        ra[2] = *reinterpret_cast<const float4*>(p.a + o1_);                                 \
        ra[3] = *reinterpret_cast<const float4*>(p.a + o1_ + 4);                             \
        vm = (v0_ ? 1 : 0) | (v1_ ? 2 : 0);                                                  \
    }
#define G3_LOAD_B(k0, stage)                                                                 \
    {                                                                                        \
        if constexpr (A2) {                                                                  \
            ra2[0] = *reinterpret_cast<const float4*>(a2p0 + (k0));                          \
            ra2[1] = *reinterpret_cast<const float4*>(a2p0 + (k0) + 4);                      \
            ra2[2] = *reinterpret_cast<const float4*>(a2p1 + (k0));                          \
            ra2[3] = *reinterpret_cast<const float4*>(a2p1 + (k0) + 4);                      \
        }                                                                                    \
        _Pragma("unroll") for (int i_ = 0; i_ < kPW; ++i_)                                   \
            glds16(p.bp + (k0), boff[i_], lds_b + (stage) * kBstage + bpiece[i_]);           \
    }
#define G3_LA(ra, vm, k0)                                                                    \
    {                                                                                        \
        if constexpr (ABF) {         \
            ra[0] = *reinterpret_cast<const float4*>(ap0 + (k0) / 2);                        \
            ra[2] = *reinterpret_cast<const float4*>(ap1 + (k0) / 2);                        \
        } else if constexpr (CV) G3_LOAD_A_CV(ra, vm, k0) else G3_LOAD_A(ra, k0)             \
    }
#define G3_WRITE(ra, vm)                                                                     \
    {                                                                                        \
        uint4 h, m, l;                                                                       \
         \
        float4 w0_ = ra[0], w1_ = ra[1], w2_ = ra[2], w3_ = ra[3];                           \
        if constexpr (CV) {                                                                  \
            const float s0_ = (vm & 1) ? 1.f : 0.f, s1_ = (vm & 2) ? 1.f : 0.f;              \
            w0_ = make_float4(w0_.x * s0_, w0_.y * s0_, w0_.z * s0_, w0_.w * s0_);           \
            w1_ = make_float4(w1_.x * s0_, w1_.y * s0_, w1_.z * s0_, w1_.w * s0_);           \
            w2_ = make_float4(w2_.x * s1_, w2_.y * s1_, w2_.z * s1_, w2_.w * s1_);           \
            w3_ = make_float4(w3_.x * s1_, w3_.y * s1_, w3_.z * s1_, w3_.w * s1_);           \
        }                                                                                    \
        if constexpr (A2) {                                                                  \
            w0_ = add4(w0_, ra2[0]); w1_ = add4(w1_, ra2[1]); w2_ = add4(w2_, ra2[2]); w3_ = add4(w3_, ra2[3]); \
        }                                                                                    \
        if constexpr (ABF) {                                                                 \
            *reinterpret_cast<float4*>(lds + (0 * 4 + akc) * kAKc + aslot0 * 16) = w0_;      \
            *reinterpret_cast<float4*>(lds + (0 * 4 + akc) * kAKc + aslot1 * 16) = w2_;      \
        } else if constexpr (H2) {                                                           \
            split8h(w0_, w1_, sc_a, &h, &l);                                                 \
            *reinterpret_cast<uint4*>(lds + (0 * 4 + akc) * kAKc + aslot0 * 16) = h;         \
            *reinterpret_cast<uint4*>(lds + (1 * 4 + akc) * kAKc + aslot0 * 16) = l;         \
            split8h(w2_, w3_, sc_a, &h, &l);                                                 \
            *reinterpret_cast<uint4*>(lds + (0 * 4 + akc) * kAKc + aslot1 * 16) = h;         \
            *reinterpret_cast<uint4*>(lds + (1 * 4 + akc) * kAKc + aslot1 * 16) = l;         \
        } else {                                                                             \
        split8(w0_, w1_, &h, &m, &l);                                                        \
        *reinterpret_cast<uint4*>(lds + (0 * 4 + akc) * kAKc + aslot0 * 16) = h;             \
        *reinterpret_cast<uint4*>(lds + (1 * 4 + akc) * kAKc + aslot0 * 16) = m;             \
        *reinterpret_cast<uint4*>(lds + (2 * 4 + akc) * kAKc + aslot0 * 16) = l;             \
        split8(w2_, w3_, &h, &m, &l);                                                        \
        *reinterpret_cast<uint4*>(lds + (0 * 4 + akc) * kAKc + aslot1 * 16) = h;             \
        *reinterpret_cast<uint4*>(lds + (1 * 4 + akc) * kAKc + aslot1 * 16) = m;             \
        *reinterpret_cast<uint4*>(lds + (2 * 4 + akc) * kAKc + aslot1 * 16) = l;             \
        }                                                                                    \
    }
#pragma unroll
    for (int i = 0; i < 4; ++i) ra2[i] = make_float4(0.f, 0.f, 0.f, 0.f);

    float sc_a = 1.f, inv_a = 1.f, inv_b = 1.f;
    if constexpr (H2) {
        float sc_b;
        h2_scale(amax_read(p.a_amax), &sc_a, &inv_a);
        h2_scale(amax_read(p.b_amax), &sc_b, &inv_b);
    }
    (void)sc_a;
    Acc<NJ> acc;
    acc.zero();

    const int a_frag = wr * 64 * 16;
    const int b_frag = kAbytes + wc * (BN / 2) * 64;

    const int nk = p.K / kBK;
    const int klast = (nk - 1) * kBK;
    int vmE = 3, vmO = 3;
    constexpr int kAloads = ABF ? 2 : 4;
#define G3_WAIT_B() { if constexpr (kAloads == 4) asm volatile("s_waitcnt vmcnt(4)" ::: "memory"); else asm volatile("s_waitcnt vmcnt(2)" ::: "memory"); }
    G3_LA(raE, vmE, 0);
    __builtin_amdgcn_sched_barrier(0);
    G3_LOAD_B(0, 0);
    __builtin_amdgcn_sched_barrier(0);
    G3_LA(raO, vmO, min(kBK, klast));
    __builtin_amdgcn_sched_barrier(0);
    for (int kt = 0; kt < nk; kt += 2) {
        __syncthreads();
        G3_WRITE(raE, vmE);
        G3_WAIT_B();
        __syncthreads();
        G3_LOAD_B(min((kt + 1) * kBK, klast), 1);
        __builtin_amdgcn_sched_barrier(0);
        G3_LA(raE, vmE, min((kt + 2) * kBK, klast));
        __builtin_amdgcn_sched_barrier(0);
        __builtin_amdgcn_s_setprio(G3_PRIO);
        if constexpr (H2) acc.template step_h2<kAKc, kBKc, true>(lds, a_frag, b_frag, lane);
        else acc.template step<kAKc, kBKc, false, ABF, true>(lds, a_frag, b_frag, lane);
        __builtin_amdgcn_s_setprio(0);
        if (kt + 1 >= nk) break;
        __syncthreads();
        G3_WRITE(raO, vmO);
        G3_WAIT_B();
        __syncthreads();
        G3_LOAD_B(min((kt + 2) * kBK, klast), 0);
        __builtin_amdgcn_sched_barrier(0);
        G3_LA(raO, vmO, min((kt + 3) * kBK, klast));
        __builtin_amdgcn_sched_barrier(0);
        __builtin_amdgcn_s_setprio(G3_PRIO);
        if constexpr (H2) acc.template step_h2<kAKc, kBKc, true>(lds, a_frag, b_frag + kBstage, lane);
        else acc.template step<kAKc, kBKc, false, ABF, true>(lds, a_frag, b_frag + kBstage, lane);
        __builtin_amdgcn_s_setprio(0);
    }
    asm volatile("s_waitcnt vmcnt(0)" ::: "memory");
#undef G3_WAIT_B

    const float omax = g3_epilogue<NJ, 4, Acc<NJ, false>, H2>(p, acc, lane, m0 + wr * 64, n0 + wc * (BN / 2), inv_a, inv_b);
    if constexpr (H2) {
        if (p.out_amax) amax_commit(p.out_amax, omax, reinterpret_cast<float*>(lds));
    }
    (void)omax;
}
#undef G3_LOAD_A
#undef G3_LOAD_A_CV
#undef G3_LA
#undef G3_LOAD_B
#undef G3_WRITE

template <int BN, bool A2, bool H2 = false>
__global__ __launch_bounds__(kThreads, 2) void gemm3_tn_kernel(G3 p)
{
    __shared__ __attribute__((aligned(16))) unsigned char lds[(H2 ? 8 : 12) * (kAKc + 2 * BN * 16)];
    const int per_xcd = (p.ntiles + 7) >> 3;
    const int tile = ((int)blockIdx.x & 7) * per_xcd + ((int)blockIdx.x >> 3);
    if (tile >= p.ntiles) return;
    const int tm = tile / p.tiles_n, tn = tile - tm * p.tiles_n;
    g3_tn_tile<BN, A2, false, false, H2>(p, lds, tm * kBM, tn * BN);
}

template <int NI, int AKC, bool F16 = false>
struct Acc2 {
    f32x4 v[2][NI][4];
    bf16x8 fa[F16 ? 1 : 3][NI];
    f16x8 fh[F16 ? 2 : 1][NI];

    __device__ __forceinline__ void zero()
    {
#pragma unroll
        for (int h = 0; h < 2; ++h)
#pragma unroll
            for (int i = 0; i < NI; ++i)
#pragma unroll
                for (int j = 0; j < 4; ++j) v[h][i][j] = f32x4{0.f, 0.f, 0.f, 0.f};
    }
    __device__ __forceinline__ void load_a(const unsigned char* lds, int a_base, int lane)
    {
        const int r16 = lane & 15, g = lane >> 4;
        const int a_frag = a_base + g * AKC + (r16 ^ (2 * g)) * 16;
        if constexpr (F16) {
#pragma unroll
            for (int pl = 0; pl < 2; ++pl)
#pragma unroll
                for (int i = 0; i < NI; ++i) fh[pl][i] = as_fragh(*reinterpret_cast<const uint4*>(lds + a_frag + pl * 4 * AKC + i * 256));
            return;
        }
#pragma unroll
        for (int pl = 0; pl < 3; ++pl)
#pragma unroll
            for (int i = 0; i < NI; ++i) fa[pl][i] = as_frag(*reinterpret_cast<const uint4*>(lds + a_frag + pl * 4 * AKC + i * 256));
    }
    template <int H>
    __device__ __forceinline__ void pass(const unsigned char* lds, int b_base, int lane)
    {
        constexpr int BKC = 128 * 16;
        const int r16 = lane & 15, g = lane >> 4;
        const int b_frag = b_base + (r16 * 4 + (g ^ ((0 - (r16 >> 2)) & 3))) * 16;
        if constexpr (F16) {
#pragma unroll
            for (int j = 0; j < 4; ++j) {
                f16x8 fb[2];
#pragma unroll
                for (int pl = 0; pl < 2; ++pl) fb[pl] = as_fragh(*reinterpret_cast<const uint4*>(lds + b_frag + pl * 4 * BKC + j * 1024));
#pragma unroll
                for (int i = 0; i < NI; ++i) v[H][i][j] = __builtin_amdgcn_mfma_f32_16x16x32_f16(fb[1], fh[0][i], v[H][i][j], 0, 0, 0);
#pragma unroll
                for (int i = 0; i < NI; ++i) v[H][i][j] = __builtin_amdgcn_mfma_f32_16x16x32_f16(fb[0], fh[1][i], v[H][i][j], 0, 0, 0);
#pragma unroll
                for (int i = 0; i < NI; ++i) v[H][i][j] = __builtin_amdgcn_mfma_f32_16x16x32_f16(fb[0], fh[0][i], v[H][i][j], 0, 0, 0);
            }
            return;
        }
#pragma unroll
        for (int j = 0; j < 4; ++j) {
            bf16x8 fb[3];
#pragma unroll
            for (int pl = 0; pl < 3; ++pl) fb[pl] = as_frag(*reinterpret_cast<const uint4*>(lds + b_frag + pl * 4 * BKC + j * 1024));
#pragma unroll
            for (int i = 0; i < NI; ++i) v[H][i][j] = __builtin_amdgcn_mfma_f32_16x16x32_bf16(fb[0], fa[2][i], v[H][i][j], 0, 0, 0);
#pragma unroll
            for (int i = 0; i < NI; ++i) v[H][i][j] = __builtin_amdgcn_mfma_f32_16x16x32_bf16(fb[2], fa[0][i], v[H][i][j], 0, 0, 0);
// ... 110 lines not shown
        } else {                                                                             \
        split8(w0_, w1_, &h, &m, &l);                                                        \
        *reinterpret_cast<uint4*>(lds + (0 * 4 + akc) * kAKcT + aslot0 * 16) = h;            \
        *reinterpret_cast<uint4*>(lds + (1 * 4 + akc) * kAKcT + aslot0 * 16) = m;            \
        *reinterpret_cast<uint4*>(lds + (2 * 4 + akc) * kAKcT + aslot0 * 16) = l;            \
        if (second) {                                                                        \
            split8(w2_, w3_, &h, &m, &l);                                                    \
            *reinterpret_cast<uint4*>(lds + (0 * 4 + akc) * kAKcT + aslot1 * 16) = h;        \
            *reinterpret_cast<uint4*>(lds + (1 * 4 + akc) * kAKcT + aslot1 * 16) = m;        \
            *reinterpret_cast<uint4*>(lds + (2 * 4 + akc) * kAKcT + aslot1 * 16) = l;        \
        }                                                                                    \
        }                                                                                    \
    }

    float sc_a = 1.f, inv_a = 1.f, inv_b = 1.f;
    if constexpr (F16) {
        float sc_b;
        h2_scale(amax_read(p.a_amax), &sc_a, &inv_a);
        h2_scale(amax_read(p.b_amax), &sc_b, &inv_b);
    }
    (void)sc_a;
    Acc2<NI, kAKcT, F16> acc;
    acc.zero();
    const int a_frag = wr * (BM / 2) * 16;
    const int b_frag = kAbytes + wc * 64 * 64;
    const int nk = p.K / kBK;
    const int klast = (nk - 1) * kBK;
    G3_LA2(0);
    __builtin_amdgcn_sched_barrier(0);
    G3_DMA2(p.bp, 0, 0);
    __builtin_amdgcn_sched_barrier(0);
    for (int kt = 0; kt < nk; ++kt) {
        __syncthreads();
        G3_WRITE2();
        __builtin_amdgcn_sched_barrier(0);
        G3_DMA2(bp1, kt * kBK, 1);
        __syncthreads();
        G3_LA2(min((kt + 1) * kBK, klast));
        __builtin_amdgcn_sched_barrier(0);
        __builtin_amdgcn_s_setprio(G3_PRIO);
        acc.load_a(lds, a_frag, lane);
        acc.template pass<0>(lds, b_frag, lane);
        __builtin_amdgcn_s_setprio(0);
        if (second) asm volatile("s_waitcnt vmcnt(4)" ::: "memory");
        else asm volatile("s_waitcnt vmcnt(2)" ::: "memory");
        __syncthreads();
        G3_DMA2(p.bp, min((kt + 1) * kBK, klast), 0);
        __builtin_amdgcn_sched_barrier(0);
        __builtin_amdgcn_s_setprio(G3_PRIO);
        acc.template pass<1>(lds, b_frag + kBstage, lane);
        __builtin_amdgcn_s_setprio(0);
    }
    asm volatile("s_waitcnt vmcnt(0)" ::: "memory");
#undef G3_LA2
#undef G3_DMA2
#undef G3_WRITE2
    float omax = 0.f;
#pragma unroll
    for (int h = 0; h < 2; ++h) {
        struct { f32x4 v[NI][4]; } out;
#pragma unroll
        for (int i = 0; i < NI; ++i)
#pragma unroll
            for (int j = 0; j < 4; ++j) out.v[i][j] = acc.v[h][i][j];
        omax = fmaxf(omax, g3_epilogue<4, NI, decltype(out), F16>(p, out, lane, m0 + wr * (BM / 2), n0 + h * 128 + wc * 64, inv_a, inv_b));
    }
    if constexpr (F16) {
        if (p.out_amax) amax_commit(p.out_amax, omax, reinterpret_cast<float*>(lds));
    }
    (void)omax;
}

template <int BN>
__global__ __launch_bounds__(kThreads, 2) void gemm3_tn_abf_kernel(G3 p)
{
    __shared__ __attribute__((aligned(16))) unsigned char lds[12 * kAKc + 2 * 12 * BN * 16];
    const int per_xcd = (p.ntiles + 7) >> 3;
    const int tile = ((int)blockIdx.x & 7) * per_xcd + ((int)blockIdx.x >> 3);
    if (tile >= p.ntiles) return;
    const int tm = tile / p.tiles_n, tn = tile - tm * p.tiles_n;
    g3_tn_tile<BN, false, false, true>(p, lds, tm * kBM, tn * BN);
}

__global__ __launch_bounds__(kThreads, 2) void gemm3_conv_kernel(G3 p)
{
    __shared__ __attribute__((aligned(16))) unsigned char lds[12 * kAKc + 2 * 12 * 128 * 16];
    const int per_xcd = (p.ntiles + 7) >> 3;
    const int tile = ((int)blockIdx.x & 7) * per_xcd + ((int)blockIdx.x >> 3);
    if (tile >= p.ntiles) return;
    const int tm = tile / p.tiles_n, tn = tile - tm * p.tiles_n;
    g3_tn_tile<128, false, true>(p, lds, tm * kBM, tn * 128);
}

template <bool A2>
__global__ __launch_bounds__(kThreads, 2) void gemm3_tn_mixed_kernel(G3 p)
{
    __shared__ __attribute__((aligned(16))) unsigned char lds[12 * kAKc + 2 * 12 * 128 * 16];
    const int g1 = ((p.ntiles + 7) >> 3) << 3;
    if ((int)blockIdx.x < g1) {
        const int per_xcd = g1 >> 3;
        const int tile = ((int)blockIdx.x & 7) * per_xcd + ((int)blockIdx.x >> 3);
        if (tile >= p.ntiles) return;
        const int tm = tile / p.tiles_n, tn = tile - tm * p.tiles_n;
        g3_tn_tile<128, A2>(p, lds, tm * kBM, tn * 128);
    } else {
        const int b = (int)blockIdx.x - g1;
        const int per_xcd = (p.ntiles2 + 7) >> 3;
        const int tile = (b & 7) * per_xcd + (b >> 3);
        if (tile >= p.ntiles2) return;
        const int tm = tile / p.tiles_n2, tn = tile - tm * p.tiles_n2;
        g3_tn_tile<64, A2>(p, lds, (p.tm0 + tm) * kBM, tn * 64);
    }
}

struct G3N {
    const float* a;
    const float* b;
    const float* b2;
    float* c;
    float* csum_a;
    float* csum_b;
    int64_t lda, ldb, ldb2;
    int R, Mdim, Ndim, b2_rows, rows_per_split, nsplit, tiles_m, tiles_n, ntiles, transpose_out;
    unsigned a_bytes, b_bytes;
    int cv_H, cv_W, cv_cin;
    int64_t c_ss, csa_ss, csb_ss;
    const float* a_amax;
    const float* b_amax;
};
constexpr int kNtGroupMax = 8;
struct G3NG {
    G3N it[kNtGroupMax];
    int tile_end[kNtGroupMax];
    int n_items, ntiles;
};

template <int BN, bool BF, bool CV, bool A16, bool B16, bool H2 = false>
__device__ __forceinline__ void gemm3_nt_tile(const G3N& p, const int tile)
{
    static_assert(!((A16 || B16) && (BF || CV || BN != 128)), "mixed-precision operands: plain 128-column tiles only");
    static_assert(!(H2 && (BF || A16 || B16)), "fp16 x 2 form: fp32 operands only");
    constexpr int NJ = BN / 32;
    constexpr int kBKc = BN * 16;
    constexpr int kPl = H2 ? 2 : 3;
    constexpr int kAbytes = kPl * 4 * kAKc;
    constexpr int kBunits = 4 * BN;
    __shared__ __attribute__((aligned(16))) unsigned char lds[kAbytes + kPl * 4 * kBKc];
    float sc_a = 1.f, sc_b = 1.f, inv_a = 1.f, inv_b = 1.f;
    if constexpr (H2) {
        h2_scale(amax_read(p.a_amax), &sc_a, &inv_a);
        h2_scale(amax_read(p.b_amax), &sc_b, &inv_b);
    }
    (void)sc_a; (void)sc_b;

    const int tn = tile % p.tiles_n, tm = (tile / p.tiles_n) % p.tiles_m, sp = tile / (p.tiles_n * p.tiles_m);
    const int m0 = tm * kBM, n0 = tn * BN;
    const int r_begin = sp * p.rows_per_split, r_end = min(p.R, r_begin + p.rows_per_split);

    const int tid = threadIdx.x, lane = tid & 63, wave = tid >> 6;
    const int wr = wave >> 1, wc = wave & 1;


    const int am = tid & 127, akc = __builtin_amdgcn_readfirstlane(tid >> 7);
    const bool a_col_ok = m0 + am < p.Mdim;
    const int acolx = min(m0 + am, p.Mdim - 1);
    int bn_[2], bkc_[2], bcolx[2];
    bool b_ok[2], b_col_ok[2];
    int b2row[2];
#pragma unroll
    for (int i = 0; i < 2; ++i) {
        const int u = tid + i * kThreads;
        b_ok[i] = u < kBunits;
        bn_[i] = u % BN;
        bkc_[i] = min(u / BN, 3);
        if (BN == 128) bkc_[i] = __builtin_amdgcn_readfirstlane(bkc_[i]);
        b_col_ok[i] = b_ok[i] && n0 + bn_[i] < p.Ndim;
        bcolx[i] = min(n0 + bn_[i], p.Ndim - 1);
        if constexpr (CV) bcolx[i] = (n0 % p.cv_cin) + bn_[i];
        b2row[i] = (!CV && p.b2) ? (r_begin + bkc_[i] * 8) % p.b2_rows : 0;
    }
    int cv_dy = 0, cv_dx = 0, cv_sh = 0, cv_x[2] = {0, 0}, cv_y[2] = {0, 0};
    if constexpr (CV) {
        const int tap = n0 / p.cv_cin;
        cv_dy = tap / 3 - 1; cv_dx = tap % 3 - 1;
        cv_sh = cv_dy * p.cv_W + cv_dx;
#pragma unroll
        for (int i = 0; i < 2; ++i) {
            const int rb = r_begin + bkc_[i] * 8;
            cv_x[i] = rb % p.cv_W;
            cv_y[i] = (rb / p.cv_W) % p.cv_H;
        }
    }
    constexpr int ESA = (BF || A16) ? 2 : 4, ESB = (BF || B16) ? 2 : 4;
    const __amdgpu_buffer_rsrc_t ars = __builtin_amdgcn_make_buffer_rsrc(const_cast<float*>(p.a), 0, p.a_bytes, 0x00020000);
    const __amdgpu_buffer_rsrc_t brs = __builtin_amdgcn_make_buffer_rsrc(const_cast<float*>(p.b), 0, p.b_bytes, 0x00020000);
    const int acolb = acolx * ESA, bcolb0 = bcolx[0] * ESB, bcolb1 = bcolx[1] * ESB;
    const int ldab = (int)p.lda * ESA, ldbb = (int)p.ldb * ESB;
    auto ld16 = [&](const __amdgpu_buffer_rsrc_t rs, int colb, int rowb, bool uniform) -> float {
        const int vo = uniform ? colb : colb + rowb, so = uniform ? rowb : 0;
        return __uint_as_float((unsigned)(unsigned short)__builtin_amdgcn_raw_buffer_load_b16(rs, vo, so, 0) << 16);
    };
    auto ld32 = [&](const __amdgpu_buffer_rsrc_t rs, int colb, int rowb, bool uniform) -> float {
        const int vo = uniform ? colb : colb + rowb, so = uniform ? rowb : 0;
        return __int_as_float(__builtin_amdgcn_raw_buffer_load_b32(rs, vo, so, 0));
    };
    auto ld = [&](const __amdgpu_buffer_rsrc_t rs, int colb, int rowb, bool uniform) -> float {
        return (BF || B16) ? ld16(rs, colb, rowb, uniform) : ld32(rs, colb, rowb, uniform);
    };
    auto lda_ = [&](const __amdgpu_buffer_rsrc_t rs, int colb, int rowb, bool uniform) -> float {
        return (BF || A16) ? ld16(rs, colb, rowb, uniform) : ld32(rs, colb, rowb, uniform);
    };
// ... 47 lines not shown
                cv_x[i] += kBK;                                                                        \
                while (cv_x[i] >= p.cv_W) { cv_x[i] -= p.cv_W; cv_y[i] = cv_y[i] + 1 == p.cv_H ? 0 : cv_y[i] + 1; } \
            }                                                                                          \
        }                                                                                              \
    }

    Acc<NJ, NJ == 4> acc;
    acc.zero();

    const int a_frag = wr * 64 * 16;
    const int b_frag = kAbytes + wc * (BN / 2) * 16;

    if (r_begin + kBK <= r_end) G3N_LOAD(r_begin, false) else G3N_LOAD(r_begin, true);
    for (int r0 = r_begin; r0 < r_end; r0 += kBK) {
        __syncthreads();
        if constexpr (H2) {
            uint4 h, l;
            split8h(make_float4(xa0[0], xa0[1], xa0[2], xa0[3]), make_float4(xa0[4], xa0[5], xa0[6], xa0[7]), sc_a, &h, &l);
            *reinterpret_cast<uint4*>(lds + (0 * 4 + akc) * kAKc + (am ^ (2 * akc)) * 16) = h;
            *reinterpret_cast<uint4*>(lds + (1 * 4 + akc) * kAKc + (am ^ (2 * akc)) * 16) = l;
            split8h(make_float4(xa1[0], xa1[1], xa1[2], xa1[3]), make_float4(xa1[4], xa1[5], xa1[6], xa1[7]), sc_a, &h, &l);
            *reinterpret_cast<uint4*>(lds + (0 * 4 + akc + 2) * kAKc + (am ^ (2 * akc + 4)) * 16) = h;
            *reinterpret_cast<uint4*>(lds + (1 * 4 + akc + 2) * kAKc + (am ^ (2 * akc + 4)) * 16) = l;
            split8h(make_float4(xb0[0], xb0[1], xb0[2], xb0[3]), make_float4(xb0[4], xb0[5], xb0[6], xb0[7]), sc_b, &h, &l);
            *reinterpret_cast<uint4*>(lds + kAbytes + (0 * 4 + bkc_[0]) * kBKc + (bn_[0] ^ (2 * bkc_[0])) * 16) = h;
            *reinterpret_cast<uint4*>(lds + kAbytes + (1 * 4 + bkc_[0]) * kBKc + (bn_[0] ^ (2 * bkc_[0])) * 16) = l;
            if (b_ok[1]) {
                split8h(make_float4(xb1[0], xb1[1], xb1[2], xb1[3]), make_float4(xb1[4], xb1[5], xb1[6], xb1[7]), sc_b, &h, &l);
                *reinterpret_cast<uint4*>(lds + kAbytes + (0 * 4 + bkc_[1]) * kBKc + (bn_[1] ^ (2 * bkc_[1])) * 16) = h;
                *reinterpret_cast<uint4*>(lds + kAbytes + (1 * 4 + bkc_[1]) * kBKc + (bn_[1] ^ (2 * bkc_[1])) * 16) = l;
            }
            if (want_csa) {
#pragma unroll
                for (int j = 0; j < 8; ++j) csa += xa0[j] + xa1[j];
            }
            if (want_csb) {
#pragma unroll
                for (int j = 0; j < 8; ++j) { csb0 += xb0[j]; csb1 += xb1[j]; }
            }
        } else {
            uint4 h, m, l;
            split8(make_float4(xa0[0], xa0[1], xa0[2], xa0[3]), make_float4(xa0[4], xa0[5], xa0[6], xa0[7]), &h, &m, &l);
            *reinterpret_cast<uint4*>(lds + (0 * 4 + akc) * kAKc + (am ^ (2 * akc)) * 16) = h;
            if (!BF && !A16) *reinterpret_cast<uint4*>(lds + (1 * 4 + akc) * kAKc + (am ^ (2 * akc)) * 16) = m;
            if (!BF && !A16) *reinterpret_cast<uint4*>(lds + (2 * 4 + akc) * kAKc + (am ^ (2 * akc)) * 16) = l;
            split8(make_float4(xa1[0], xa1[1], xa1[2], xa1[3]), make_float4(xa1[4], xa1[5], xa1[6], xa1[7]), &h, &m, &l);
            *reinterpret_cast<uint4*>(lds + (0 * 4 + akc + 2) * kAKc + (am ^ (2 * akc + 4)) * 16) = h;
            if (!BF && !A16) *reinterpret_cast<uint4*>(lds + (1 * 4 + akc + 2) * kAKc + (am ^ (2 * akc + 4)) * 16) = m;
            if (!BF && !A16) *reinterpret_cast<uint4*>(lds + (2 * 4 + akc + 2) * kAKc + (am ^ (2 * akc + 4)) * 16) = l;
            split8(make_float4(xb0[0], xb0[1], xb0[2], xb0[3]), make_float4(xb0[4], xb0[5], xb0[6], xb0[7]), &h, &m, &l);
            *reinterpret_cast<uint4*>(lds + kAbytes + (0 * 4 + bkc_[0]) * kBKc + (bn_[0] ^ (2 * bkc_[0])) * 16) = h;
            if (!BF && !B16) *reinterpret_cast<uint4*>(lds + kAbytes + (1 * 4 + bkc_[0]) * kBKc + (bn_[0] ^ (2 * bkc_[0])) * 16) = m;
            if (!BF && !B16) *reinterpret_cast<uint4*>(lds + kAbytes + (2 * 4 + bkc_[0]) * kBKc + (bn_[0] ^ (2 * bkc_[0])) * 16) = l;
            if (b_ok[1]) {
                split8(make_float4(xb1[0], xb1[1], xb1[2], xb1[3]), make_float4(xb1[4], xb1[5], xb1[6], xb1[7]), &h, &m, &l);
                *reinterpret_cast<uint4*>(lds + kAbytes + (0 * 4 + bkc_[1]) * kBKc + (bn_[1] ^ (2 * bkc_[1])) * 16) = h;
                if (!BF && !B16) *reinterpret_cast<uint4*>(lds + kAbytes + (1 * 4 + bkc_[1]) * kBKc + (bn_[1] ^ (2 * bkc_[1])) * 16) = m;
                if (!BF && !B16) *reinterpret_cast<uint4*>(lds + kAbytes + (2 * 4 + bkc_[1]) * kBKc + (bn_[1] ^ (2 * bkc_[1])) * 16) = l;
            }
            if (want_csa) {
#pragma unroll
                for (int j = 0; j < 8; ++j) csa += xa0[j] + xa1[j];
            }
            if (want_csb) {
#pragma unroll
                for (int j = 0; j < 8; ++j) { csb0 += xb0[j]; csb1 += xb1[j]; }
            }
        }
        __syncthreads();
        if (r0 + 2 * kBK <= r_end) G3N_LOAD(r0 + kBK, false) else if (r0 + kBK < r_end) G3N_LOAD(r0 + kBK, true);
        __builtin_amdgcn_s_setprio(G3_PRIO);
        if constexpr (H2) acc.template step_h2<kAKc, kBKc>(lds, a_frag, b_frag, lane);
        else if constexpr (A16 || B16) acc.template step<kAKc, kBKc, false, A16, B16>(lds, a_frag, b_frag, lane);
        else acc.template step<kAKc, kBKc, BF>(lds, a_frag, b_frag, lane);
        __builtin_amdgcn_s_setprio(0);
    }

    float* cp = p.c + (int64_t)sp * p.c_ss;
    acc.quads(lane, [&](int mo, int no, float4 o) {
        const int m = m0 + wr * 64 + mo, n = n0 + wc * (BN / 2) + no;
        if (m >= p.Mdim) return;
        if constexpr (H2) o = make_float4(o.x * inv_a * inv_b, o.y * inv_a * inv_b, o.z * inv_a * inv_b, o.w * inv_a * inv_b);
        const float e4[4] = {o.x, o.y, o.z, o.w};
        if (!p.transpose_out) {
            if (n + 3 < p.Ndim) {
                *reinterpret_cast<float4*>(cp + (int64_t)m * p.Ndim + n) = o;
            } else {
#pragma unroll
                for (int e = 0; e < 4; ++e)
                    if (n + e < p.Ndim) cp[(int64_t)m * p.Ndim + n + e] = e4[e];
            }
        } else {
#pragma unroll
            for (int e = 0; e < 4; ++e)
                if (n + e < p.Ndim) cp[(int64_t)(n + e) * p.Mdim + m] = e4[e];
        }
    });
    if (want_csa || want_csb) {
        __syncthreads();
        float* red = reinterpret_cast<float*>(lds);
        for (int i = tid; i < kBM + BN; i += kThreads) red[i] = 0.f;
        __syncthreads();
        if (want_csa) atomicAdd(&red[am], csa);
        if (want_csb) {
            atomicAdd(&red[kBM + bn_[0]], csb0);
            if (b_ok[1]) atomicAdd(&red[kBM + bn_[1]], csb1);
        }
        __syncthreads();
        if (want_csa && tid < kBM && m0 + tid < p.Mdim) p.csum_a[(int64_t)sp * p.csa_ss + m0 + tid] = red[tid];
        if (want_csb && tid < BN && n0 + tid < p.Ndim) p.csum_b[(int64_t)sp * p.csb_ss + n0 + tid] = red[kBM + tid];
    }
    (void)a_col_ok; (void)b_col_ok;
}

template <int BN, bool BF = false, bool CV = false, bool A16 = false, bool B16 = false, bool H2 = false>
__global__ __launch_bounds__(kThreads, 2) void gemm3_nt_kernel(G3N p)
{
    const int per_xcd = (p.ntiles + 7) >> 3;
    const int tile = ((int)blockIdx.x & 7) * per_xcd + ((int)blockIdx.x >> 3);
    if (tile >= p.ntiles) return;
    gemm3_nt_tile<BN, BF, CV, A16, B16, H2>(p, tile);
}

template <bool H2>
__global__ __launch_bounds__(kThreads, 2) void gemm3_nt_group_kernel(G3NG g)
{
    const int per_xcd = (g.ntiles + 7) >> 3;
    const int tile = ((int)blockIdx.x & 7) * per_xcd + ((int)blockIdx.x >> 3);
    if (tile >= g.ntiles) return;
    int i = 0;
    while (i + 1 < g.n_items && tile >= g.tile_end[i]) ++i;
    const int first = i ? g.tile_end[i - 1] : 0;
    gemm3_nt_tile<128, false, false, false, false, H2>(g.it[i], tile - first);
}

#include "gemm3_nt2.h"

__global__ __launch_bounds__(256) void gemm3_split_kernel(const float* __restrict__ w, unsigned short* __restrict__ out,
                                                          int R, int C, int transpose)
{
    const int64_t total = (int64_t)R * C;
    for (int64_t i = (int64_t)blockIdx.x * blockDim.x + threadIdx.x; i < total; i += (int64_t)gridDim.x * blockDim.x) {
        int r, c;
        if (transpose) { c = (int)(i / R); r = (int)(i - (int64_t)c * R); } else { r = (int)(i / C); c = (int)(i - (int64_t)r * C); }
        const float x = w[(int64_t)r * C + c];
        const unsigned xb = __float_as_uint(x);
        const float r1 = x - __uint_as_float(xb & 0xFFFF0000u);
        const unsigned rb = __float_as_uint(r1);
        const float r2 = r1 - __uint_as_float(rb & 0xFFFF0000u);
        const unsigned lb = __float_as_uint(r2) + 0x8000u;
        out[i] = (unsigned short)(xb >> 16);
        out[total + i] = (unsigned short)(rb >> 16);
        out[2 * total + i] = (unsigned short)(lb >> 16);
    }
}

__global__ __launch_bounds__(256) void gemm3_split_grouped_kernel(const MpfSplitItem* __restrict__ items, int n_items)
{
    int lo = 0, hi = n_items - 1;
    const int64_t blk = blockIdx.x;
    while (lo < hi) {
        const int mid = (lo + hi + 1) >> 1;
        if (items[mid].first_block <= blk) lo = mid; else hi = mid - 1;
    }
    const MpfSplitItem it = items[lo];
    const float* __restrict__ w = it.src;
// ... 105 lines not shown
    if (n <= 0) return 0;
    if ((uintptr_t)x & 15) return mpf::fail(MPF_E_SHAPE, "amax_f32: x must be 16-byte aligned");
    const int64_t n4 = n / 4;
    const int blocks = (int)std::min<int64_t>(1024, std::max<int64_t>(1, (n4 + 1023) / 1024));
    mpf::prof_begin((hipStream_t)stream);
    mpf::set_kernel("amax_kernel");
    hipLaunchKernelGGL(amax_kernel, dim3(blocks), dim3(256), 0, (hipStream_t)stream, x, n4, n, amax);
    mpf::prof_end("amax_kernel", (hipStream_t)stream, 4.0 * (double)n);
    return mpf::check(hipGetLastError(), "mpf_amax_f32");
}

__global__ __launch_bounds__(256) void h2_range_stats_kernel(const float* __restrict__ a, int rows, int cols, int64_t lda,
                                                             const float* __restrict__ amax_slot, int log2_below,
                                                             unsigned long long* __restrict__ counters)
{
    const int lane = threadIdx.x & 63, wave = threadIdx.x >> 6;
    const float ref = __uint_as_float(amax_read(amax_slot));
    const float thr = ldexpf(ref, -log2_below);
    unsigned nz = 0, below = 0;
    for (int r = blockIdx.x * 4 + wave; r < rows; r += gridDim.x * 4) {
        const float4* __restrict__ row = reinterpret_cast<const float4*>(a + (int64_t)r * lda);
        float m = 0.f;
        for (int c = lane; c < cols / 4; c += 64) {
            const float4 v = row[c];
            m = fmaxf(fmaxf(m, fmaxf(fabsf(v.x), fabsf(v.y))), fmaxf(fabsf(v.z), fabsf(v.w)));
        }
#pragma unroll
        for (int o = 32; o >= 1; o >>= 1) m = fmaxf(m, __shfl_xor(m, o));
        nz += m > 0.f;
        below += (m > 0.f && m < thr);
    }
    __shared__ unsigned red[8];
    if (lane == 0) { red[wave * 2] = nz; red[wave * 2 + 1] = below; }
    __syncthreads();
    if (threadIdx.x < 2) {
        const unsigned v = red[threadIdx.x] + red[2 + threadIdx.x] + red[4 + threadIdx.x] + red[6 + threadIdx.x];
        if (v) atomicAdd(counters + threadIdx.x, (unsigned long long)v);
    }
}

extern "C" int mpf_h2_range_stats(const float* a, int rows, int cols, int64_t lda, const float* amax_slot, int log2_below,
                                  unsigned long long* counters_device, void* stream)
{
    if (!a || !amax_slot || !counters_device) return mpf::fail(MPF_E_NULL, "h2_range_stats: NULL buffer");
    if (rows <= 0 || cols <= 0 || cols % 4 || lda < cols || lda % 4 || ((uintptr_t)a & 15) || log2_below < 0 || log2_below > 120)
        return mpf::fail(MPF_E_SHAPE, "h2_range_stats: cols and lda must be multiples of 4, a 16-byte aligned, 0 <= log2_below <= 120");
    const int blocks = std::min(2048, (rows + 3) / 4);
    mpf::set_kernel("h2_range_stats_kernel");
    hipLaunchKernelGGL(h2_range_stats_kernel, dim3(blocks), dim3(256), 0, (hipStream_t)stream, a, rows, cols, lda, amax_slot, log2_below,
                       counters_device);
    return mpf::check(hipGetLastError(), "mpf_h2_range_stats");
}

extern "C" int mpf_amax_f32_grouped(const MpfAmaxItem* items_device, int n_items, int64_t total_blocks, void* stream)
{
    if (n_items == 0 || total_blocks == 0) return 0;
    if (!items_device) return mpf::fail(MPF_E_NULL, "amax_f32_grouped: NULL table");
    if (n_items < 0 || total_blocks < 0 || total_blocks > 0x7fffffffLL) return mpf::fail(MPF_E_SHAPE, "amax_f32_grouped: bad sizes");
    mpf::set_kernel("amax_grouped_kernel");
    hipLaunchKernelGGL(amax_grouped_kernel, dim3((unsigned)total_blocks), dim3(256), 0, (hipStream_t)stream, items_device, n_items);
    return mpf::check(hipGetLastError(), "mpf_amax_f32_grouped");
}

extern "C" int mpf_gemm3_split_grouped_h2(const MpfSplitItemH2* items_device, int n_items, int64_t total_blocks, void* stream)
{
    if (n_items == 0 || total_blocks == 0) return 0;
    if (!items_device) return mpf::fail(MPF_E_NULL, "gemm3_split_grouped_h2: NULL table");
    if (n_items < 0 || total_blocks < 0 || total_blocks > 0x7fffffffLL) return mpf::fail(MPF_E_SHAPE, "gemm3_split_grouped_h2: bad sizes");
    mpf::set_kernel("gemm3_split_grouped_h2_kernel");
    hipLaunchKernelGGL(gemm3_split_grouped_h2_kernel, dim3((unsigned)total_blocks), dim3(256), 0, (hipStream_t)stream, items_device,
                       n_items);
    return mpf::check(hipGetLastError(), "mpf_gemm3_split_grouped_h2");
}

int mpf::set_gemm3_option(const char* key, int v)
{
    if (!strcmp(key, "gemm3_mixed_tiles")) { g_mixed = v; return 0; }
    if (!strcmp(key, "gemm3_two_pass")) { g_two_pass = v; return 0; }
    if (!strcmp(key, "gemm3_two_pass_rows")) { g_two_pass_rows = v; return 0; }
    if (!strcmp(key, "gemm3_ws")) { g_ws = v; return 0; }
    if (!strcmp(key, "gemm3_tn3")) { g_tn3 = v; return 0; }
    if (!strcmp(key, "gemm3_tn3_176")) { g_tn3_176 = v; return 0; }
    if (!strcmp(key, "gemm3_nt2")) { g_nt2 = v; return 0; }
    if (strcmp(key, "gemm3_ablate") != 0) return 1;
    g_ablate = v;
    return 0;
}

extern "C" int mpf_gemm3_split(const float* w, int rows, int cols, int transpose, void* planes, void* stream)
{
    hipStream_t st = (hipStream_t)stream;
    if (!w || !planes) return mpf::fail(MPF_E_NULL, "gemm3_split: NULL buffer");
    if (rows <= 0 || cols <= 0) return mpf::fail(MPF_E_SHAPE, "gemm3_split: bad sizes");
    const int64_t total = (int64_t)rows * cols;
    const int blocks = (int)((total + 255) / 256 < 2048 ? (total + 255) / 256 : 2048);
    mpf::set_kernel("gemm3_split_kernel");
    hipLaunchKernelGGL(gemm3_split_kernel, dim3(blocks), dim3(256), 0, st, w, (unsigned short*)planes, rows, cols, transpose);
    return mpf::check(hipGetLastError(), "mpf_gemm3_split");
}

extern "C" int mpf_gemm3_split_grouped(const MpfSplitItem* items_device, int n_items, int64_t total_blocks, void* stream)
{
    if (n_items == 0 || total_blocks == 0) return 0;
    if (!items_device) return mpf::fail(MPF_E_NULL, "gemm3_split_grouped: NULL table");
    if (n_items < 0 || total_blocks < 0 || total_blocks > 0x7fffffffLL) return mpf::fail(MPF_E_SHAPE, "gemm3_split_grouped: bad sizes");
    mpf::set_kernel("gemm3_split_grouped_kernel");
    hipLaunchKernelGGL(gemm3_split_grouped_kernel, dim3((unsigned)total_blocks), dim3(256), 0, (hipStream_t)stream, items_device,
                       n_items);
    return mpf::check(hipGetLastError(), "mpf_gemm3_split_grouped");
}

namespace {

struct Route {
    const void* fn = nullptr;
    const char* name = nullptr;
    const char* what = nullptr;
    int threads = kThreads;
    int blocks = 0;
    size_t lds = 0;
    mpf::LdsAttr* attr = nullptr;
    double w_el = 6.0;
    int arg[2] = {0, 0};
};

struct Work { double bytes, flops; };

template <typename P>
int g3_launch(const Route& r, const P& p, hipStream_t st, const Work w)
{
    if (r.lds)
        if (int e = mpf::ensure_dynamic_lds(r.fn, r.lds, *r.attr)) return e;
    mpf::prof_begin(st);
    mpf::set_kernel(r.name);
    void* args[] = {(void*)&p, (void*)&r.arg[0], (void*)&r.arg[1]};
    if (hipError_t e = hipLaunchKernel(r.fn, dim3(r.blocks), dim3(r.threads), args, r.lds, st); e != hipSuccess) return mpf::check(e, r.what);
    mpf::prof_end(r.name, st, w.bytes, w.flops);
    return mpf::check(hipGetLastError(), r.what);
}

constexpr int round8(int tiles) { return (tiles + 7) / 8 * 8; }
constexpr int cdiv(int a, int b) { return (a + b - 1) / b; }
inline int g3_slots() { return 2 * mpf::cu_count(); }

struct ColTile { int bn, tiles_n; };
inline ColTile g3_col_tile(int N)
{
    const int t128 = cdiv(N, 128), t96 = cdiv(N, 96);
    return t96 * 96 < t128 * 128 ? ColTile{96, t96} : ColTile{128, t128};
}


int g3_fill(G3& p, const char* who, const void* a, int64_t lda, const void* planes, const float* bias, int64_t ldc, int M, int N, int K)
{
    const float* consts = nullptr;
    if (int rc = g3_consts(&consts, who)) return rc;
    p = G3{};
    p.a = (const float*)a; p.lda = lda; p.bp = (const unsigned short*)planes; p.plane = (int64_t)N * K; p.ldc = ldc;
    p.M = M; p.N = N; p.K = K;
    p.bias = bias ? bias : consts; p.bias_cm = bias ? 1 : 0;
    p.cin = p.cin2 = consts; p.gate = consts + 4;
    p.gbits = reinterpret_cast<const unsigned char*>(consts + 8);
    p.cv_sign = 1;
    p.t3_bm = kT3BM;
    return 0;
}

inline void g3_operand(const float*& slot, int64_t& ld, int& cm, const float* v, int64_t ldv)
{
    if (v) { slot = v; ld = ldv; cm = 1; }
}

inline Work g3_tn_work(const G3& p, const Route& r, double a_el = 4.0)
{
    const double M = p.M, N = p.N, K = p.K;
    return {a_el * M * (p.cv_cin ? p.cv_cin : p.K) + (p.c16 ? 2.0 : 4.0) * M * N + r.w_el * N * K, 2.0 * M * N * K};
}

Route g3_ws_route(const G3& p)
{
    static const struct { int key; const void* fn; } kEpilogues[] = {
        {0, (const void*)gemm3_ws_kernel<0, false, false, false>},  {8, (const void*)gemm3_ws_kernel<1, false, false, false>},
        {2, (const void*)gemm3_ws_kernel<0, false, true, false>},   {10, (const void*)gemm3_ws_kernel<1, false, true, false>},
        {3, (const void*)gemm3_ws_kernel<0, false, true, true>},    {4, (const void*)gemm3_ws_kernel<0, true, false, false>},
        {12, (const void*)gemm3_ws_kernel<1, true, false, false>}};
    static mpf::LdsAttr attr[sizeof(kEpilogues) / sizeof(kEpilogues[0])];
    const int key = (p.cin_cm ? 8 : 0) | (p.gbits_cm ? 4 : 0) | (p.relu ? 2 : 0) | (p.gbits_out ? 1 : 0);
    Route r;
    for (size_t i = 0; i < sizeof(kEpilogues) / sizeof(kEpilogues[0]); ++i) {
        if (kEpilogues[i].key != key) continue;
        const int ncg = p.N / 256;
        int per_xcd = mpf::cu_count() / 8 / ncg * ncg;
        if (per_xcd < ncg) per_xcd = ncg;
        int workers = per_xcd / ncg * 8;
        const int tiles16 = cdiv(p.M, 16);
        if (workers > tiles16) workers = round8(tiles16);
        r.fn = kEpilogues[i].fn; r.name = "gemm3_tn_kernel<h2 ws>"; r.what = "mpf_gemm3_tn_h2(ws)";
        r.threads = kWsThreads; r.lds = kWsLds; r.attr = &attr[i]; r.w_el = 4.0;
        r.blocks = workers * ncg;
        r.arg[0] = cdiv(cdiv(p.M, workers), 16) * 16;
        r.arg[1] = ncg;
    }
    return r;
}

Route g3_tn_route(G3& p, bool a_bf16, const char* what)
{
    const bool h2 = p.a_amax != nullptr, a2 = p.a2 != nullptr, a_al16 = ((uintptr_t)p.a & 15) == 0;
    const int M = p.M, N = p.N;
    const ColTile ct = g3_col_tile(N);
    const int tiles_m = cdiv(M, kBM);
    p.tiles_n = ct.tiles_n;
    p.ntiles = tiles_m * ct.tiles_n;
    Route r;
    r.what = what;
    r.w_el = h2 ? 4.0 : 6.0;
    if (h2 && !a2 && !p.gate_cm && !p.cin2_cm && g_ws > 0 && N >= g_ws && p.K == kWsK && N % 256 == 0 && a_al16) {
        const Route ws = g3_ws_route(p);
        if (ws.fn) return ws;
    }
    if (h2 && !a2 && g_tn3 && N % 256 == 0 && M >= 2048 && a_al16 && p.lda % 4 == 0) {
        const int cus = mpf::cu_count(), nt3 = cdiv(M, kT3BM) * (N / 256), rem = nt3 % cus;
        if (g_tn3 == 2 || (nt3 >= cus * 3 / 4 && (rem == 0 || 4 * rem >= 3 * cus || nt3 >= 4 * cus))) {
            const int nt176 = cdiv(M, 176) * (N / 256);
            static mpf::LdsAttr attr;
            if (g_tn3_176 && cdiv(nt176, cus) <= cdiv(nt3, cus)) p.t3_bm = 176;
            p.tiles_n = N / 256;
            p.ntiles = cdiv(M, p.t3_bm) * p.tiles_n;
            r.fn = (const void*)gemm3_tn3_kernel;
            r.name = p.t3_bm == kT3BM ? "gemm3_tn_kernel<h2 192x256>" : "gemm3_tn_kernel<h2 192x256:176>";
            r.what = "mpf_gemm3_tn_h2(192x256)";
            r.threads = kT3T; r.lds = kT3Lds; r.attr = &attr;
            r.blocks = round8(p.ntiles);
            return r;
        }
    }
    if (!a2 && !a_bf16 && g_two_pass > 0 && N % 256 == 0 && N >= g_two_pass) {
        const int slots = g3_slots();
        p.tiles_n = N / 256;
        const int t128 = cdiv(M, 128) * p.tiles_n, t96 = cdiv(M, 96) * p.tiles_n;
        const bool rows96 = g_two_pass_rows == 96 || (g_two_pass_rows == 0 && cdiv(t96, slots) * 96 < cdiv(t128, slots) * 128);
        p.ntiles = rows96 ? t96 : t128;
        if (h2) {
            r.fn = rows96 ? (const void*)gemm3_tn2_kernel<96, false, true> : (const void*)gemm3_tn2_kernel<128, false, true>;
            r.name = rows96 ? "gemm3_tn_kernel<h2 96x256>" : "gemm3_tn_kernel<h2 128x256>";
// ... 448 lines not shown
    if (q >= cq + sq) return;
    if (q < cq) {
        const float* src = c_part + 2 * q;
        float2 acc = make_float2(0.f, 0.f);
        int sp = 0;
        for (; sp + 8 <= nsplit; sp += 8) {
            float2 t[8];
#pragma unroll
            for (int k = 0; k < 8; ++k) t[k] = *reinterpret_cast<const float2*>(src + (int64_t)(sp + k) * cn);
#pragma unroll
            for (int k = 0; k < 8; ++k) { acc.x += t[k].x; acc.y += t[k].y; }
        }
        for (; sp < nsplit; ++sp) {
            const float2 t = *reinterpret_cast<const float2*>(src + (int64_t)sp * cn);
            acc.x += t.x; acc.y += t.y;
        }
        *reinterpret_cast<float2*>(c_out + 2 * q) = acc;
        return;
    }
    const int64_t j = 2 * (q - cq);
    float2 acc[4] = {make_float2(0.f, 0.f), make_float2(0.f, 0.f), make_float2(0.f, 0.f), make_float2(0.f, 0.f)};
    int sp = 0;
    for (; sp + 8 <= nsplit; sp += 8) {
        float2 t[8];
        int lv[8];
#pragma unroll
        for (int k = 0; k < 8; ++k) {
            t[k] = *reinterpret_cast<const float2*>(s_part + (int64_t)(sp + k) * sn + j);
            lv[k] = (int)level_of_split[sp + k];
        }
#pragma unroll
        for (int k = 0; k < 8; ++k)
#pragma unroll
            for (int l = 0; l < 4; ++l) {
                acc[l].x += lv[k] == l ? t[k].x : 0.f;
                acc[l].y += lv[k] == l ? t[k].y : 0.f;
            }
    }
    for (; sp < nsplit; ++sp) {
        const float2 t = *reinterpret_cast<const float2*>(s_part + (int64_t)sp * sn + j);
        const int lv = (int)level_of_split[sp];
#pragma unroll
        for (int l = 0; l < 4; ++l) {
            acc[l].x += lv == l ? t.x : 0.f;
            acc[l].y += lv == l ? t.y : 0.f;
        }
    }
    float2 tot = make_float2(0.f, 0.f);
#pragma unroll
    for (int l = 0; l < 4; ++l)
        if (l < L) {
            *reinterpret_cast<float2*>(lvl_out + (int64_t)l * sn + j) = acc[l];
            tot.x += acc[l].x; tot.y += acc[l].y;
        }
    *reinterpret_cast<float2*>(s_out + j) = tot;
}

extern "C" int mpf_gemm3_nt_reduce_levels(const float* c_part, int64_t c_numel, const float* s_part, int64_t s_numel, int nsplit,
                                          const int64_t* level_of_split, int n_levels, float* c_out, float* lvl_out, float* s_out,
                                          void* stream)
{
    if (!c_part || !c_out || !s_part || !s_out || !lvl_out || !level_of_split) return mpf::fail(MPF_E_NULL, "gemm3_nt_reduce_levels: NULL buffer");
    if (nsplit <= 0 || c_numel <= 0 || s_numel <= 0 || c_numel % 4 || s_numel % 4 || n_levels < 1 || n_levels > 4)
        return mpf::fail(MPF_E_SHAPE, "gemm3_nt_reduce_levels: sizes must be positive multiples of 4, 1..4 levels");
    const int64_t quads = (c_numel + s_numel) / 2;
    mpf::set_kernel("nt_reduce_levels_kernel");
    hipLaunchKernelGGL(nt_reduce_levels_kernel, dim3((unsigned)((quads + 255) / 256)), dim3(256), 0, (hipStream_t)stream, c_part, c_numel,
                       s_part, s_numel, nsplit, level_of_split, n_levels, c_out, lvl_out, s_out);
    return mpf::check(hipGetLastError(), "mpf_gemm3_nt_reduce_levels");
}

extern "C" int mpf_gemm3_nt_reduce(const float* c_part, int64_t c_numel, const float* s_part, int64_t s_numel, int nsplit,
                                   float* c_out, float* s_out, void* stream)
{
    if (!c_part || !c_out || (s_numel > 0 && (!s_part || !s_out))) return mpf::fail(MPF_E_NULL, "gemm3_nt_reduce: NULL buffer");
    if (nsplit <= 0 || c_numel <= 0 || s_numel < 0 || c_numel % 4 || s_numel % 4)
        return mpf::fail(MPF_E_SHAPE, "gemm3_nt_reduce: sizes must be positive multiples of 4");
    const int64_t quads = (c_numel + s_numel) / 2;
    mpf::set_kernel("nt_reduce_kernel");
    hipLaunchKernelGGL(nt_reduce_kernel<true>, dim3((unsigned)((quads + 255) / 256)), dim3(256), 0, (hipStream_t)stream, c_part,
                       c_numel, s_part, s_numel, nsplit, c_out, s_out);
    return mpf::check(hipGetLastError(), "mpf_gemm3_nt_reduce");
}
```

Before: 86.16 images/sec.

## Route backbone stride-1 conv backward through native bf16 GEMM kernels with fused ReLU gate

Adds a custom autograd path for stride-1 channels-last bf16 ResNet convolutions that computes the data and weight gradients with in-house GEMM kernels instead of MIOpen's convolution_backward. The ReLU threshold_backward of the following bias_act is folded into the data-gradient epilogue through a gate. Per-stage transposed weights for the data gradient are built lazily with one grouped transpose kernel. A route table limits which shapes use it, and split-K partial sums are reduced for the weight gradient. This adds per-layer host bookkeeping and extra workspace, and the gate handoff between layers is subtle to get right.

```diff
diff --git a/include/mpformer_hip.h b/include/mpformer_hip.h
--- a/include/mpformer_hip.h
+++ b/include/mpformer_hip.h
@@ -437,6 +437,19 @@
 int mpf_maxpool3x3s2_forward(const void* x, void* y, void* code, int N, int H, int W, int C, void* stream);
 int mpf_maxpool3x3s2_backward(const void* gy, const void* code, void* gx, int N, int H, int W, int C, void* stream);
 
+size_t mpf_conv_bwd_bf16_workspace_bytes(int n_img, int H, int W, int Cin, int Cout, int ksize);
+int mpf_conv_bwd_bf16_parts(int n_img, int H, int W, int Cin, int Cout, int ksize, int stride, int pad, int dilation, int groups,
+                            int dtype, int channel_last);
+int mpf_conv_bwd_bf16(const void* dy, const void* x, const void* wt, const void* gate, void* dx, void* dw, void* workspace,
+                      size_t workspace_bytes, int n_img, int H, int W, int Cin, int Cout, int ksize, int stride, int pad, int dilation,
+                      int groups, int dtype, int channel_last, void* stream);
+typedef struct MpfDgradWeightItem {
+    const void* src;
+    void* dst;
+    int64_t cout, cin, k, s_co, s_ci, s_ky, s_kx, first_block;
+} MpfDgradWeightItem;
+int mpf_grouped_dgrad_weights(const MpfDgradWeightItem* items_device, int n_items, int64_t total_blocks, void* stream);
+
 int mpf_upload_small(const void* host_src, void* device_dst, int64_t nbytes, void* stream);
 
 int mpf_res_ln256_forward(const float* x, const void* t, int t_dtype, const float* gamma, const float* beta,
diff --git a/mp_former_amd/_lib.py b/mp_former_amd/_lib.py
--- a/mp_former_amd/_lib.py
+++ b/mp_former_amd/_lib.py
@@ -140,6 +140,10 @@
     "mpf_mask_loss_finalize_backward": (_c_int, [_c_vp, _c_vp, _c_vp, _c_int, _c_int, _c_int, _c_vp, _c_vp, _c_vp]),
     "mpf_bias_act": (_c_int, [_c_vp, _c_vp, _c_vp, _c_vp, ctypes.c_int64, _c_int, _c_int, _c_int, _c_vp]),
     "mpf_relu_bwd_add": (_c_int, [_c_vp, _c_vp, _c_vp, _c_vp, ctypes.c_int64, _c_int, _c_vp]),
+    "mpf_conv_bwd_bf16_workspace_bytes": (ctypes.c_size_t, [_c_int] * 6),
+    "mpf_conv_bwd_bf16_parts": (_c_int, [_c_int] * 12),
+    "mpf_conv_bwd_bf16": (_c_int, [_c_vp] * 7 + [ctypes.c_size_t] + [_c_int] * 12 + [_c_vp]),
+    "mpf_grouped_dgrad_weights": (_c_int, [_c_vp, _c_int, ctypes.c_int64, _c_vp]),
     "mpf_maxpool3x3s2_forward": (_c_int, [_c_vp] * 3 + [_c_int] * 4 + [_c_vp]),
     "mpf_maxpool3x3s2_backward": (_c_int, [_c_vp] * 3 + [_c_int] * 4 + [_c_vp]),
     "mpf_upload_small": (_c_int, [_c_vp, _c_vp, ctypes.c_int64, _c_vp]),
@@ -280,6 +284,19 @@
         check(code, name)
 
 
+def call_answer(name, device, *args):
+    fn = _status_fns.get(name) or _status_fn(name)
+    idx = device.index
+    if idx is None or idx == torch.cuda.current_device():
+        code = fn(*args)
+    else:
+        with torch.cuda.device(device):
+            code = fn(*args)
+    if code < 0:
+        check(code, name)
+    return code
+
+
 def ptr(t):
     return None if t is None else t.data_ptr()
 
diff --git a/mp_former_amd/backbone.py b/mp_former_amd/backbone.py
--- a/mp_former_amd/backbone.py
+++ b/mp_former_amd/backbone.py
@@ -35,25 +35,34 @@
         return x * scale.to(x.dtype).view(1, -1, 1, 1) + bias.to(x.dtype).view(1, -1, 1, 1)
 
 
+class _Gate:
+    __slots__ = ("armed", "fused")
+
+    def __init__(self):
+        self.armed = self.fused = False
+
+
 class _BiasAct(torch.autograd.Function):
 
     @staticmethod
-    def forward(ctx, x, shift, res, relu):
+    def forward(ctx, x, shift, res, relu, gate=None):
         y = torch.empty_like(x)
         C = x.shape[1]
         _lib.call("mpf_bias_act", x.device, x.data_ptr(), shift.data_ptr(), _lib.ptr(res), y.data_ptr(), x.numel(), C,
                   _lib.DTYPE[x.dtype], 1 if relu else 0, _lib.stream_ptr(x.device))
-        ctx.relu, ctx.has_res = relu, res is not None
+        ctx.relu, ctx.has_res, ctx.gate = relu, res is not None, gate
         if relu:
             ctx.save_for_backward(y)
+            if gate is not None:
+                gate.armed = True
         return y
 
     @staticmethod
     def backward(ctx, g):
-        if ctx.relu:
+        if ctx.relu and not (ctx.gate is not None and ctx.gate.fused):
             (y,) = ctx.saved_tensors
             g = torch.ops.aten.threshold_backward(g, y, 0)
-        return g, None, (g if ctx.has_res else None), None
+        return g, None, (g if ctx.has_res else None), None, None
 
 
 def _relu_bwd_add(ga, gb, y):
@@ -96,9 +105,9 @@
                                  and res.is_contiguous(memory_format=torch.channels_last))))
 
 
-def bias_act(x, shift, res=None, relu=True):
+def bias_act(x, shift, res=None, relu=True, gate=None):
     if _bias_act_ok(x, res):
-        return _BiasAct.apply(x, shift, res, relu)
+        return _BiasAct.apply(x, shift, res, relu, gate)
     y = x + shift.to(x.dtype).view(1, -1, 1, 1)
     if res is not None:
         y = y + res
@@ -145,14 +154,137 @@
     return F.max_pool2d(x, kernel_size=3, stride=2, padding=1)
 
 
-def conv_bn(conv, bn, x, folded=None, res=None, relu=True, fork=False):
+_bwd_parts_cache = {}
+
+
+def _conv_geometry(x, w, conv):
+    if x.dim() != 4 or w.dim() != 4 or w.shape[2] != w.shape[3]:
+        return None
+    st, pd, dl = conv.stride, conv.padding, conv.dilation
+    if not (isinstance(pd, tuple) and st[0] == st[1] and pd[0] == pd[1] and dl[0] == dl[1]):
+        return None
+    N, C, H, W = x.shape
+    cl = x.is_contiguous(memory_format=torch.channels_last) and not (x.is_contiguous() and C > 1 and H * W > 1)
+    dt = _lib.DTYPE.get(x.dtype, -1) if x.dtype == w.dtype else -1
+    return (N, H, W, C if w.shape[1] == C else 0, w.shape[0], w.shape[2], st[0], pd[0], dl[0], conv.groups, dt, 1 if cl else 0)
+
+
+def _bwd_parts(geo, device):
+    key = (geo, device, _lib.option_generation())
+    r = _bwd_parts_cache.get(key)
+    if r is None:
+        if len(_bwd_parts_cache) > 512:
+            _bwd_parts_cache.clear()
+        N, H, W, Cin, Cout, k = geo[:6]
+        lib = _lib.lib()
+        parts = int(lib.mpf_conv_bwd_bf16_parts(*geo)) if Cin > 0 else 0
+        r = _bwd_parts_cache[key] = (parts, int(lib.mpf_conv_bwd_bf16_workspace_bytes(N, H, W, Cin, Cout, k)) if parts & 2 else 0)
+    return r
+
+
+class _StageDgradWeights:
+
+    def __init__(self):
+        self.ws, self.out = [], None
+
+    def add(self, w):
+        self.ws.append(w.detach())
+        return len(self.ws) - 1
+
+    def get(self, i):
+        if self.out is None:
+            self.out = _grouped_dgrad_weights(self.ws)
+        return self.out[i]
+
+
+_gdw_layouts = {}
+
+
+def _grouped_dgrad_weights(ws):
+    dev = ws[0].device
+    key = tuple((t.shape, t.stride()) for t in ws)
+    lay = _gdw_layouts.get(key)
+    if lay is None:
+        table = np.zeros((len(ws), 10), dtype=np.int64)
+        offs, tot, blk = [], 0, 0
+        for i, t in enumerate(ws):
+            co, ci, k, _ = t.shape
+            assert t.dtype == torch.bfloat16 and _dense(t)
+            table[i, 2:] = (co, ci, k, t.stride(0), t.stride(1), t.stride(2), t.stride(3), blk)
+            offs.append(tot)
+            tot += (t.numel() + 63) & ~63
+            blk += k * k * ((co + 63) // 64) * ((ci + 63) // 64)
+        lay = (table, np.asarray(offs, dtype=np.int64) * 2, tot, blk, [(o, t.shape[1], t.shape[2] ** 2 * t.shape[0]) for o, t in zip(offs, ws)])
+        if len(_gdw_layouts) > 64:
+            _gdw_layouts.clear()
+        _gdw_layouts[key] = lay
+    table, offs_b, tot, blk, views = lay
+    out = torch.empty(tot, dtype=torch.bfloat16, device=dev)
+    table[:, 0] = [t.data_ptr() for t in ws]
+    table[:, 1] = offs_b + out.data_ptr()
+    items = upload(table.reshape(-1), dev)
+    _lib.call("mpf_grouped_dgrad_weights", dev, items.data_ptr(), len(ws), blk, _lib.stream_ptr(dev))
+    return [out[o:o + r * c].view(r, c) for o, r, c in views]
+
+
+class _ConvNativeBwd(torch.autograd.Function):
+
+    @staticmethod
+    def forward(ctx, x, w, conv, geo, gated, wts, wt_index):
+        ctx.save_for_backward(x, w)
+        ctx.conv, ctx.geo, ctx.gated, ctx.wts, ctx.wt_index = conv, geo, gated, wts, wt_index
+        return F.conv2d(x, w, None, conv.stride, conv.padding, conv.dilation, conv.groups)
+
+    @staticmethod
+    def backward(ctx, gy):
+        x, w = ctx.saved_tensors
+        conv = ctx.conv
+        N, H, W, Cin, Cout, k, st, pd, dl, groups, dt, cl = ctx.geo
+        need_x, need_w = ctx.needs_input_grad[0], ctx.needs_input_grad[1]
+        dev = x.device
+        served, dx, dw = 0, None, None
+        if gy.dtype == x.dtype and gy.is_contiguous(memory_format=torch.channels_last):
+            parts, ws_bytes = _bwd_parts(ctx.geo, dev)
+            want_x, want_w = need_x and parts & 1 and ctx.wt_index >= 0, need_w and parts & 2
+            if want_x or want_w:
+                stream = _lib.stream_ptr(dev)
+                work = _lib.scratch("conv_bwd_bf16", dev, stream, ws_bytes) if (want_w and ws_bytes) else None
+                dx = torch.empty_like(x) if want_x else None
+                dw_cl = torch.empty((Cout, k, k, Cin), dtype=w.dtype, device=dev) if want_w else None
+                served = _lib.call_answer("mpf_conv_bwd_bf16", dev, gy.data_ptr(), x.data_ptr(),
+                                          ctx.wts.get(ctx.wt_index).data_ptr() if want_x else None, x.data_ptr() if ctx.gated else None,
+                                          _lib.ptr(dx), _lib.ptr(dw_cl), _lib.ptr(work), work.numel() if work is not None else 0,
+                                          N, H, W, Cin, Cout, k, st, pd, dl, groups, dt, cl, stream)
+                dw = dw_cl.permute(0, 3, 1, 2) if want_w else None
+        miss_x, miss_w = need_x and not served & 1, need_w and not served & 2
+        if miss_x or miss_w:
+            gx, gw, _ = torch.ops.aten.convolution_backward(gy, x, w, None, conv.stride, conv.padding, conv.dilation, False, [0, 0],
+                                                            conv.groups, [bool(miss_x), bool(miss_w), False])
+            if miss_x:
+                dx = torch.ops.aten.threshold_backward(gx, x, 0) if ctx.gated else gx
+            if miss_w:
+                dw = gw
+        return (dx if need_x else None), (dw if need_w else None), None, None, None, None, None
+
+
+def conv_bn(conv, bn, x, folded=None, res=None, relu=True, fork=False, wts=None, take_gate=None, hand_gate=None):
     if folded is not None:
         w, shift = folded
     else:
         scale, shift = bn.scale_bias()
         w = conv.weight * scale.view(-1, 1, 1, 1)
-    y = F.conv2d(x, w, None, conv.stride, conv.padding, conv.dilation, conv.groups)
-    return bias_act_fork(y, shift, res) if fork else bias_act(y, shift, res, relu)
+    y = None
+    if wts is not None and x.is_cuda and torch.is_grad_enabled() and (x.requires_grad or w.requires_grad):
+        geo = _conv_geometry(x, w, conv)
+        parts = _bwd_parts(geo, x.device)[0] if geo is not None else 0
+        if parts:
+            gated = bool(parts & 1) and take_gate is not None and take_gate.armed and x.requires_grad
+            if gated:
+                take_gate.fused = True
+            y = _ConvNativeBwd.apply(x, w, conv, geo, gated, wts, wts.add(w) if parts & 1 else -1)
+    if y is None:
+        y = F.conv2d(x, w, None, conv.stride, conv.padding, conv.dilation, conv.groups)
+    return bias_act_fork(y, shift, res) if fork else bias_act(y, shift, res, relu, hand_gate)
 
 
 def _dense(t):
@@ -253,17 +385,18 @@
             self.__dict__["_pairs"] = p
         return p
 
-    def forward(self, x, fw=None):
-        return self.forward_fork((x, x), fw)[0]
-
-    def forward_fork(self, xs, fw=None):
+    def forward(self, x, fw=None, wts=None):
+        return self.forward_fork((x, x), fw, wts)[0]
+
+    def forward_fork(self, xs, fw=None, wts=None):
         f = fw if fw is not None else [None] * 4
         x_main, x_skip = xs
         p = self.pairs()
-        out = conv_bn(p[0][0], p[0][1], x_main, f[0])
-        out = conv_bn(p[1][0], p[1][1], out, f[1])
-        sc = x_skip if len(p) == 3 else conv_bn(p[3][0], p[3][1], x_skip, f[3], relu=False)
-        return conv_bn(p[2][0], p[2][1], out, f[2], res=sc, fork=True)
+        g1, g2 = _Gate(), _Gate()
+        out = conv_bn(p[0][0], p[0][1], x_main, f[0], wts=wts, hand_gate=g1)
+        out = conv_bn(p[1][0], p[1][1], out, f[1], wts=wts, take_gate=g1, hand_gate=g2)
+        sc = x_skip if len(p) == 3 else conv_bn(p[3][0], p[3][1], x_skip, f[3], relu=False, wts=wts)
+        return conv_bn(p[2][0], p[2][1], out, f[2], res=sc, fork=True, wts=wts, take_gate=g2)
 
 
 class ResNet50(nn.Module):
@@ -311,9 +444,10 @@
         folded = ResNet50._fold_group([p for b in blocks for p in b.pairs()], dtype)
         k = 0
         xs = x if isinstance(x, tuple) else (x, x)
+        wts = _StageDgradWeights() if dtype == torch.bfloat16 else None
         for b in blocks:
             n = len(b.pairs())
-            xs = b.forward_fork(xs, folded[k:k + n])
+            xs = b.forward_fork(xs, folded[k:k + n], wts)
             k += n
         x = xs
         out[name] = xs[0]
diff --git a/mp_former_amd/csrc/elementwise.hip b/mp_former_amd/csrc/elementwise.hip
--- a/mp_former_amd/csrc/elementwise.hip
+++ b/mp_former_amd/csrc/elementwise.hip
@@ -749,6 +749,52 @@
 
 namespace {
 
+__global__ __launch_bounds__(256) void grouped_dgrad_weights_kernel(const MpfDgradWeightItem* __restrict__ items, int n_items)
+{
+    __shared__ unsigned short tile[64][66];
+    int lo = 0, hi = n_items - 1;
+    const int64_t blk = blockIdx.x;
+    while (lo < hi) {
+        const int mid = (lo + hi + 1) >> 1;
+        if (items[mid].first_block <= blk) lo = mid; else hi = mid - 1;
+    }
+    const MpfDgradWeightItem it = items[lo];
+    const unsigned short* __restrict__ src = static_cast<const unsigned short*>(it.src);
+    unsigned short* __restrict__ dst = static_cast<unsigned short*>(it.dst);
+    const int tco = (int)((it.cout + 63) / 64), tci = (int)((it.cin + 63) / 64);
+    const int b = (int)(blk - it.first_block);
+    const int tap = b / (tco * tci), rest = b - tap * (tco * tci);
+    const int co0 = (rest / tci) * 64, ci0 = (rest % tci) * 64;
+    const int ky = tap / (int)it.k, kx = tap - ky * (int)it.k;
+    const int tx = threadIdx.x & 63, ty = threadIdx.x >> 6;
+#pragma unroll 4
+    for (int r = 0; r < 16; ++r) {
+        const int co = co0 + ty + 4 * r, ci = ci0 + tx;
+        if (co < it.cout && ci < it.cin) tile[ty + 4 * r][tx] = src[co * it.s_co + ci * it.s_ci + ky * it.s_ky + kx * it.s_kx];
+    }
+    __syncthreads();
+    const int64_t ldd = it.k * it.k * it.cout;
+#pragma unroll 4
+    for (int r = 0; r < 16; ++r) {
+        const int ci = ci0 + ty + 4 * r, co = co0 + tx;
+        if (co < it.cout && ci < it.cin) dst[ci * ldd + (int64_t)tap * it.cout + co] = tile[tx][ty + 4 * r];
+    }
+}
+
+}
+
+extern "C" int mpf_grouped_dgrad_weights(const MpfDgradWeightItem* items_device, int n_items, int64_t total_blocks, void* stream)
+{
+    if (n_items == 0 || total_blocks == 0) return 0;
+    if (!items_device) return mpf::fail(MPF_E_NULL, "grouped_dgrad_weights: NULL table");
+    if (n_items < 0 || total_blocks < 0 || total_blocks > 0x7fffffffLL) return mpf::fail(MPF_E_SHAPE, "grouped_dgrad_weights: bad sizes");
+    mpf::set_kernel("grouped_dgrad_weights_kernel");
+    hipLaunchKernelGGL(grouped_dgrad_weights_kernel, dim3((unsigned)total_blocks), dim3(256), 0, (hipStream_t)stream, items_device, n_items);
+    return mpf::check(hipGetLastError(), "mpf_grouped_dgrad_weights");
+}
+
+namespace {
+
 constexpr int kOptBlock = 2048;
 
 __device__ __forceinline__ const MpfOptItem& opt_item_of(const MpfOptItem* __restrict__ items, int n_items, int64_t blk)
diff --git a/mp_former_amd/csrc/gemm3.hip b/mp_former_amd/csrc/gemm3.hip
--- a/mp_former_amd/csrc/gemm3.hip
+++ b/mp_former_amd/csrc/gemm3.hip
@@ -44,6 +44,9 @@
     int64_t ldgbits, ldgbits_out;
     int gbits_cm;
     int t3_bm;
+    const unsigned short* gate16;
+    int64_t ldgate16;
+    int gate16_cm;
 };
 
 int g_ablate = 0;
@@ -54,6 +57,8 @@
 int g_tn3 = 1;
 int g_tn3_176 = 1;
 int g_ws = 512;
+int g_bb_native = 1;
+int g_bb_rps = 0;
 
 
 __device__ __forceinline__ unsigned pack_hi16(unsigned a, unsigned b)
@@ -338,8 +343,9 @@
     }
 };
 
-__device__ __attribute__((aligned(16))) unsigned g3_const[12] = {0u, 0u, 0u, 0u, 0x3f800000u, 0x3f800000u, 0x3f800000u, 0x3f800000u,
-                                    0xffffffffu, 0xffffffffu, 0xffffffffu, 0xffffffffu};
+__device__ __attribute__((aligned(16))) unsigned g3_const[16] = {0u, 0u, 0u, 0u, 0x3f800000u, 0x3f800000u, 0x3f800000u, 0x3f800000u,
+                                    0xffffffffu, 0xffffffffu, 0xffffffffu, 0xffffffffu,
+                                    0x3f803f80u, 0x3f803f80u, 0x3f803f80u, 0x3f803f80u};
 
 int g3_consts(const float** out, const char* who)
 {
@@ -358,7 +364,7 @@
     return 0;
 }
 
-template <int NJ, int NI = 4, typename AccT = Acc<NJ, false>, bool SCALED = false, bool PIPE = false>
+template <int NJ, int NI = 4, typename AccT = Acc<NJ, false>, bool SCALED = false, bool PIPE = false, bool G16 = false>
 __device__ __forceinline__ float g3_epilogue(const G3& p, const AccT& acc, int lane, int m_wave, int n_wave, const float inv_a = 1.f,
                                             const float inv_b = 1.f, const int m_end = 0x7fffffff)
 {
@@ -373,7 +379,9 @@
         const int m = m_wave + i * 16 + r16;
         mok[i] = m < p.M && m < m_end;
         mrow[i] = min(m, p.M - 1);
-        if constexpr (NJ <= 2) {
+        if constexpr (G16) {
+            gb[i] = make_uint2(0u, 0u);
+        } else if constexpr (NJ <= 2) {
             gb[i].x = *reinterpret_cast<const unsigned*>(p.gbits + mrow[i] * p.ldgbits + (n_wave >> 3) * p.gbits_cm);
             gb[i].y = 0u;
         } else {
@@ -381,15 +389,19 @@
         }
         wb[i][0] = wb[i][1] = 0u;
     }
-    struct Ops { float4 bz, ci[NI], c2[NI], gt[NI]; };
+    struct Ops { float4 bz, ci[NI], c2[NI], gt[NI]; uint2 g16[NI]; };
     auto load_ops = [&](const int j, Ops& q) {
         const int nc = min(n_wave + j * 16 + g * 4, p.N - 4);
         q.bz = *reinterpret_cast<const float4*>(p.bias + nc * p.bias_cm);
 #pragma unroll
         for (int i = 0; i < NI; ++i) {
-            q.ci[i] = *reinterpret_cast<const float4*>(p.cin + mrow[i] * p.ldcin + nc * p.cin_cm);
-            q.c2[i] = *reinterpret_cast<const float4*>(p.cin2 + mrow[i] * p.ldcin2 + nc * p.cin2_cm);
-            q.gt[i] = *reinterpret_cast<const float4*>(p.gate + mrow[i] * p.ldgate + nc * p.gate_cm);
+            if constexpr (G16) {
+                q.g16[i] = *reinterpret_cast<const uint2*>(p.gate16 + mrow[i] * p.ldgate16 + nc * p.gate16_cm);
+            } else {
+                q.ci[i] = *reinterpret_cast<const float4*>(p.cin + mrow[i] * p.ldcin + nc * p.cin_cm);
+                q.c2[i] = *reinterpret_cast<const float4*>(p.cin2 + mrow[i] * p.ldcin2 + nc * p.cin2_cm);
+                q.gt[i] = *reinterpret_cast<const float4*>(p.gate + mrow[i] * p.ldgate + nc * p.gate_cm);
+            }
         }
     };
     Ops ops[2];
@@ -414,15 +426,23 @@
             if constexpr (SCALED)
                 o = make_float4(o.x * inv_a * inv_b, o.y * inv_a * inv_b, o.z * inv_a * inv_b, o.w * inv_a * inv_b);
             o = make_float4(o.x + bz.x, o.y + bz.y, o.z + bz.z, o.w + bz.w);
-            o = make_float4(o.x + ci[i].x, o.y + ci[i].y, o.z + ci[i].z, o.w + ci[i].w);
-            o = make_float4(o.x + c2[i].x, o.y + c2[i].y, o.z + c2[i].z, o.w + c2[i].w);
+            if constexpr (!G16) {
+                o = make_float4(o.x + ci[i].x, o.y + ci[i].y, o.z + ci[i].z, o.w + ci[i].w);
+                o = make_float4(o.x + c2[i].x, o.y + c2[i].y, o.z + c2[i].z, o.w + c2[i].w);
+            }
             if (p.relu) o = make_float4(fmaxf(o.x, 0.f), fmaxf(o.y, 0.f), fmaxf(o.z, 0.f), fmaxf(o.w, 0.f));
-            o = make_float4(gt[i].x > 0.f ? o.x : 0.f, gt[i].y > 0.f ? o.y : 0.f, gt[i].z > 0.f ? o.z : 0.f, gt[i].w > 0.f ? o.w : 0.f);
-            if (p.gbits_cm) {
+            if constexpr (!G16)
+                o = make_float4(gt[i].x > 0.f ? o.x : 0.f, gt[i].y > 0.f ? o.y : 0.f, gt[i].z > 0.f ? o.z : 0.f, gt[i].w > 0.f ? o.w : 0.f);
+            if constexpr (G16) {
+                const uint2 gq = ops[j & 1].g16[i];
+                o = make_float4(__uint_as_float(gq.x << 16) <= 0.f ? 0.f : o.x, __uint_as_float(gq.x & 0xffff0000u) <= 0.f ? 0.f : o.y,
+                                __uint_as_float(gq.y << 16) <= 0.f ? 0.f : o.z, __uint_as_float(gq.y & 0xffff0000u) <= 0.f ? 0.f : o.w);
+            }
+            if (!G16 && p.gbits_cm) {
                 const unsigned nib = ((j & 2) ? gb[i].y : gb[i].x) >> ((j & 1) * 16 + g * 4);
                 o = make_float4((nib & 1u) ? o.x : 0.f, (nib & 2u) ? o.y : 0.f, (nib & 4u) ? o.z : 0.f, (nib & 8u) ? o.w : 0.f);
             }
-            if (p.gbits_out) {
+            if (!G16 && p.gbits_out) {
                 const unsigned pos = (o.x > 0.f ? 1u : 0u) | (o.y > 0.f ? 2u : 0u) | (o.z > 0.f ? 4u : 0u) | (o.w > 0.f ? 8u : 0u);
                 wb[i][(j >> 1) & 1] |= pos << ((j & 1) * 16 + g * 4);
             }
@@ -444,7 +464,7 @@
             }
         }
     }
-    if (p.gbits_out) {
+    if (!G16 && p.gbits_out) {
 #pragma unroll
         for (int i = 0; i < NI; ++i) {
             unsigned lo = wb[i][0], hi = wb[i][1];
@@ -469,18 +489,19 @@
 #include "gemm3_ws.h"
 #include "gemm3_tn3.h"
 
-template <int BN, bool A2, bool CV = false, bool ABF = false, bool H2 = false>
+template <int BN, bool A2, bool CV = false, bool ABF = false, bool H2 = false, bool B1 = false>
 __device__ __forceinline__ void g3_tn_tile(const G3& p, unsigned char* lds, const int m0, const int n0)
 {
-    static_assert(!(ABF && (A2 || CV)), "bf16 A: no addend, no convolution mode");
+    static_assert(!(ABF && (A2 || (CV && !B1))), "bf16 A: no addend; convolution mode only in the pure-bf16 form");
     static_assert(!(H2 && (ABF || A2)), "fp16 x 2 form: fp32 A, no addend rows");
+    static_assert(!B1 || ABF, "one-plane B: bf16 A only");
     constexpr int NJ = BN / 32;
     constexpr int kBKc = BN * 16;
     constexpr int kPl = H2 ? 2 : 3;
-    constexpr int kAbytes = kPl * 4 * kAKc;
+    constexpr int kAbytes = (B1 ? 1 : kPl) * 4 * kAKc;
     constexpr int kBunits = 3 * BN * 4;
     constexpr int kBiter = (kBunits + kThreads - 1) / kThreads;
-    constexpr int kBstage = kPl * 4 * kBKc;
+    constexpr int kBstage = (B1 ? 1 : kPl) * 4 * kBKc;
     constexpr int kPieces = kBstage / 1024;
     constexpr int kPW = (kPieces + 3) / 4;
 
@@ -562,7 +583,18 @@
     }
 #define G3_LA(ra, vm, k0)                                                                    \
     {                                                                                        \
-        if constexpr (ABF) {         \
+        if constexpr (ABF && CV) {   \
+            const int tap_ = (k0) / p.cv_cin, kk_ = (k0) - tap_ * p.cv_cin;                  \
+            const int dy_ = (tap_ / 3 - 1) * p.cv_sign, dx_ = (tap_ % 3 - 1) * p.cv_sign;    \
+            const int sh_ = dy_ * p.cv_W + dx_;                                              \
+            const bool v0_ = (unsigned)(cy0 + dy_) < (unsigned)p.cv_H && (unsigned)(cx0 + dx_) < (unsigned)p.cv_W; \
+            const bool v1_ = (unsigned)(cy1 + dy_) < (unsigned)p.cv_H && (unsigned)(cx1 + dx_) < (unsigned)p.cv_W; \
+            const unsigned o0_ = (unsigned)(min(max(mr0 + sh_, 0), p.M - 1) * (int)p.lda + akc * 8 + kk_); \
+            const unsigned o1_ = (unsigned)(min(max(mr1 + sh_, 0), p.M - 1) * (int)p.lda + akc * 8 + kk_); \
+            ra[0] = *reinterpret_cast<const float4*>(reinterpret_cast<const unsigned short*>(p.a) + o0_); \
+            ra[2] = *reinterpret_cast<const float4*>(reinterpret_cast<const unsigned short*>(p.a) + o1_); \
+            vm = (v0_ ? 1 : 0) | (v1_ ? 2 : 0);                                              \
+        } else if constexpr (ABF) {  \
             ra[0] = *reinterpret_cast<const float4*>(ap0 + (k0) / 2);                        \
             ra[2] = *reinterpret_cast<const float4*>(ap1 + (k0) / 2);                        \
         } else if constexpr (CV) G3_LOAD_A_CV(ra, vm, k0) else G3_LOAD_A(ra, k0)             \
@@ -572,7 +604,11 @@
         uint4 h, m, l;                                                                       \
          \
         float4 w0_ = ra[0], w1_ = ra[1], w2_ = ra[2], w3_ = ra[3];                           \
-        if constexpr (CV) {                                                                  \
+        if constexpr (CV && ABF) {                   \
+            const bool k0_ = vm & 1, k1_ = vm & 2;                                           \
+            w0_ = make_float4(k0_ ? w0_.x : 0.f, k0_ ? w0_.y : 0.f, k0_ ? w0_.z : 0.f, k0_ ? w0_.w : 0.f); \
+            w2_ = make_float4(k1_ ? w2_.x : 0.f, k1_ ? w2_.y : 0.f, k1_ ? w2_.z : 0.f, k1_ ? w2_.w : 0.f); \
+        } else if constexpr (CV) {                                                           \
             const float s0_ = (vm & 1) ? 1.f : 0.f, s1_ = (vm & 2) ? 1.f : 0.f;              \
             w0_ = make_float4(w0_.x * s0_, w0_.y * s0_, w0_.z * s0_, w0_.w * s0_);           \
             w1_ = make_float4(w1_.x * s0_, w1_.y * s0_, w1_.z * s0_, w1_.w * s0_);           \
@@ -641,7 +677,7 @@
         __builtin_amdgcn_sched_barrier(0);
         __builtin_amdgcn_s_setprio(G3_PRIO);
         if constexpr (H2) acc.template step_h2<kAKc, kBKc, true>(lds, a_frag, b_frag, lane);
-        else acc.template step<kAKc, kBKc, false, ABF, true>(lds, a_frag, b_frag, lane);
+        else acc.template step<kAKc, kBKc, B1, ABF && !B1, true>(lds, a_frag, b_frag, lane);
         __builtin_amdgcn_s_setprio(0);
         if (kt + 1 >= nk) break;
         __syncthreads();
@@ -654,13 +690,13 @@
         __builtin_amdgcn_sched_barrier(0);
         __builtin_amdgcn_s_setprio(G3_PRIO);
         if constexpr (H2) acc.template step_h2<kAKc, kBKc, true>(lds, a_frag, b_frag + kBstage, lane);
-        else acc.template step<kAKc, kBKc, false, ABF, true>(lds, a_frag, b_frag + kBstage, lane);
+        else acc.template step<kAKc, kBKc, B1, ABF && !B1, true>(lds, a_frag, b_frag + kBstage, lane);
         __builtin_amdgcn_s_setprio(0);
     }
     asm volatile("s_waitcnt vmcnt(0)" ::: "memory");
 #undef G3_WAIT_B
 
-    const float omax = g3_epilogue<NJ, 4, Acc<NJ, false>, H2>(p, acc, lane, m0 + wr * 64, n0 + wc * (BN / 2), inv_a, inv_b);
+    const float omax = g3_epilogue<NJ, 4, Acc<NJ, false>, H2, false, B1>(p, acc, lane, m0 + wr * 64, n0 + wc * (BN / 2), inv_a, inv_b);
     if constexpr (H2) {
         if (p.out_amax) amax_commit(p.out_amax, omax, reinterpret_cast<float*>(lds));
     }
@@ -937,6 +973,17 @@
     g3_tn_tile<BN, false, false, true>(p, lds, tm * kBM, tn * BN);
 }
 
+template <int BN, bool CV>
+__global__ __launch_bounds__(kThreads, 3) void gemm3_tn_bf16_kernel(G3 p)
+{
+    __shared__ __attribute__((aligned(16))) unsigned char lds[4 * kAKc + 2 * 4 * BN * 16];
+    const int per_xcd = (p.ntiles + 7) >> 3;
+    const int tile = ((int)blockIdx.x & 7) * per_xcd + ((int)blockIdx.x >> 3);
+    if (tile >= p.ntiles) return;
+    const int tm = tile / p.tiles_n, tn = tile - tm * p.tiles_n;
+    g3_tn_tile<BN, false, CV, true, false, true>(p, lds, tm * kBM, tn * BN);
+}
+
 __global__ __launch_bounds__(kThreads, 2) void gemm3_conv_kernel(G3 p)
 {
     __shared__ __attribute__((aligned(16))) unsigned char lds[12 * kAKc + 2 * 12 * 128 * 16];
@@ -982,6 +1029,8 @@
     int64_t c_ss, csa_ss, csb_ss;
     const float* a_amax;
     const float* b_amax;
+    unsigned short* c16;
+    int64_t ldc16;
 };
 constexpr int kNtGroupMax = 8;
 struct G3NG {
@@ -1195,6 +1244,17 @@
         if (m >= p.Mdim) return;
         if constexpr (H2) o = make_float4(o.x * inv_a * inv_b, o.y * inv_a * inv_b, o.z * inv_a * inv_b, o.w * inv_a * inv_b);
         const float e4[4] = {o.x, o.y, o.z, o.w};
+        if constexpr (BF) {
+            if (p.c16) {
+#pragma unroll
+                for (int e = 0; e < 4; ++e) {
+                    unsigned u = __float_as_uint(e4[e]);
+                    u += 0x7fffu + ((u >> 16) & 1u);
+                    if (n + e < p.Ndim) p.c16[(int64_t)m * p.ldc16 + n + e] = (unsigned short)(u >> 16);
+                }
+                return;
+            }
+        }
         if (!p.transpose_out) {
             if (n + 3 < p.Ndim) {
                 *reinterpret_cast<float4*>(cp + (int64_t)m * p.Ndim + n) = o;
@@ -1466,6 +1526,8 @@
     if (!strcmp(key, "gemm3_tn3")) { g_tn3 = v; return 0; }
     if (!strcmp(key, "gemm3_tn3_176")) { g_tn3_176 = v; return 0; }
     if (!strcmp(key, "gemm3_nt2")) { g_nt2 = v; return 0; }
+    if (!strcmp(key, "backbone_bwd_native")) { if (v < 0 || v > 2) return mpf::fail(MPF_E_SHAPE, "backbone_bwd_native: 0, 1 or 2"); g_bb_native = v; return 0; }
+    if (!strcmp(key, "backbone_bwd_rps")) { if (v < 0) return mpf::fail(MPF_E_SHAPE, "backbone_bwd_rps: must not be negative"); g_bb_rps = v; return 0; }
     if (strcmp(key, "gemm3_ablate") != 0) return 1;
     g_ablate = v;
     return 0;
@@ -1545,6 +1607,7 @@
     p.bias = bias ? bias : consts; p.bias_cm = bias ? 1 : 0;
     p.cin = p.cin2 = consts; p.gate = consts + 4;
     p.gbits = reinterpret_cast<const unsigned char*>(consts + 8);
+    p.gate16 = reinterpret_cast<const unsigned short*>(consts + 12);
     p.cv_sign = 1;
     p.t3_bm = kT3BM;
     return 0;
@@ -2159,3 +2222,5 @@
                        c_numel, s_part, s_numel, nsplit, c_out, s_out);
     return mpf::check(hipGetLastError(), "mpf_gemm3_nt_reduce");
 }
+
+#include "gemm3_convbwd.h"
diff --git a/mp_former_amd/csrc/gemm3_convbwd.h b/mp_former_amd/csrc/gemm3_convbwd.h
--- /dev/null
+++ b/mp_former_amd/csrc/gemm3_convbwd.h
@@ -0,0 +1,122 @@
+#pragma once
+
+namespace {
+
+struct BbRoute { int ks, cin, cout, rows, parts, rps; };
+constexpr BbRoute kBbRoutes[] = {
+    {1, 64, 64, 131072, 1, 0},
+    {3, 64, 64, 131072, 1, 0},
+    {1, 64, 256, 131072, 1, 0},
+    {1, 128, 512, 32768, 1, 0},
+    {3, 128, 128, 32768, 3, 608},
+    {1, 256, 1024, 8192, 1, 0},
+    {1, 1024, 256, 8192, 1, 0},
+    {3, 256, 256, 8192, 3, 608},
+    {1, 1024, 512, 8192, 1, 0},
+    {1, 512, 2048, 2048, 1, 0},
+    {1, 2048, 512, 2048, 1, 0},
+    {3, 512, 512, 2048, 2, 704},
+};
+
+struct BbPlan { int parts, rps, nsplit; };
+
+inline int bb_rule_rps(int ks, int Cin, int Cout, int rows)
+{
+    const int tiles = cdiv(Cout, kBM) * cdiv(ks * ks * Cin, 128);
+    const int ns = std::max(1, g3_slots() / tiles);
+    return std::max(kBK, cdiv(cdiv(rows, ns), kBK) * kBK);
+}
+
+BbPlan bb_plan(int ks, int Cin, int Cout, int64_t rows64, int W)
+{
+    BbPlan pl{0, 0, 0};
+    if (g_bb_native == 0 || (ks != 1 && ks != 3) || Cin <= 0 || Cout <= 0 || Cin % 32 != 0 || Cout % 32 != 0 || rows64 <= 0) return pl;
+    if (rows64 * std::max(Cin, Cout) >= (1ll << 31) || (int64_t)ks * ks * Cin * Cout >= (1ll << 30)) return pl;
+    const int rows = (int)rows64;
+    const int servable = 1 | ((ks == 1 || (W % 8 == 0 && Cin % 128 == 0)) ? 2 : 0);
+    if (g_bb_native >= 2) {
+        pl.parts = servable;
+    } else {
+        for (const BbRoute& r : kBbRoutes)
+            if (r.ks == ks && r.cin == Cin && r.cout == Cout && r.rows == rows) { pl.parts = r.parts & servable; pl.rps = r.rps; }
+    }
+    if (g_bb_rps > 0) pl.rps = cdiv(g_bb_rps, kBK) * kBK;
+    if (pl.rps <= 0) pl.rps = bb_rule_rps(ks, Cin, Cout, rows);
+    pl.nsplit = cdiv(rows, pl.rps);
+    return pl;
+}
+
+}
+
+extern "C" size_t mpf_conv_bwd_bf16_workspace_bytes(int n_img, int H, int W, int Cin, int Cout, int ksize)
+{
+    const BbPlan pl = bb_plan(ksize, Cin, Cout, (int64_t)n_img * H * W, W);
+    if (!(pl.parts & 2) || pl.nsplit <= 1) return 0;
+    return (size_t)pl.nsplit * Cout * ksize * ksize * Cin * sizeof(float);
+}
+
+extern "C" int mpf_conv_bwd_bf16_parts(int n_img, int H, int W, int Cin, int Cout, int ksize, int stride, int pad, int dilation,
+                                       int groups, int dtype, int channel_last)
+{
+    if (dtype != MPF_BF16 || !channel_last || stride != 1 || dilation != 1 || groups != 1 || pad != ksize / 2 || n_img <= 0 || H <= 0 ||
+        W <= 0)
+        return 0;
+    return bb_plan(ksize, Cin, Cout, (int64_t)n_img * H * W, W).parts;
+}
+
+extern "C" int mpf_conv_bwd_bf16(const void* dy, const void* x, const void* wt, const void* gate, void* dx, void* dw, void* workspace,
+                                 size_t workspace_bytes, int n_img, int H, int W, int Cin, int Cout, int ksize, int stride, int pad,
+                                 int dilation, int groups, int dtype, int channel_last, void* stream)
+{
+    const int served = mpf_conv_bwd_bf16_parts(n_img, H, W, Cin, Cout, ksize, stride, pad, dilation, groups, dtype, channel_last);
+    const BbPlan pl = bb_plan(ksize, Cin, Cout, (int64_t)n_img * H * W, W);
+    const int parts = served & ((dx ? 1 : 0) | (dw ? 2 : 0));
+    if (!parts) return 0;
+    if (!dy || ((parts & 1) && !wt) || ((parts & 2) && !x)) return mpf::fail(MPF_E_NULL, "conv_bwd_bf16: NULL buffer");
+    if (((uintptr_t)dy | (uintptr_t)x | (uintptr_t)wt | (uintptr_t)gate | (uintptr_t)dx | (uintptr_t)dw) & 15)
+        return mpf::fail(MPF_E_SHAPE, "conv_bwd_bf16: buffers must be 16-byte aligned");
+    const int rows = n_img * H * W, taps = ksize * ksize;
+    hipStream_t st = (hipStream_t)stream;
+    if (parts & 1) {
+        G3 p;
+        if (int rc = g3_fill(p, "conv_bwd_bf16: constants", dy, Cout, wt, nullptr, Cin, rows, Cin, taps * Cout)) return rc;
+        p.c16 = (unsigned short*)dx;
+        if (gate) { p.gate16 = (const unsigned short*)gate; p.ldgate16 = Cin; p.gate16_cm = 1; }
+        if (ksize == 3) { p.cv_H = H; p.cv_W = W; p.cv_cin = Cout; p.cv_sign = -1; }
+        const int bn = Cin <= 64 ? 64 : 128;
+        p.tiles_n = cdiv(Cin, bn);
+        p.ntiles = cdiv(rows, kBM) * p.tiles_n;
+        Route r;
+        r.fn = ksize == 3 ? (bn == 64 ? (const void*)gemm3_tn_bf16_kernel<64, true> : (const void*)gemm3_tn_bf16_kernel<128, true>)
+                          : (bn == 64 ? (const void*)gemm3_tn_bf16_kernel<64, false> : (const void*)gemm3_tn_bf16_kernel<128, false>);
+        r.name = "conv_bwd_data_bf16"; r.what = "mpf_conv_bwd_bf16(data)"; r.w_el = 2.0;
+        r.blocks = round8(p.ntiles);
+        if (int rc = g3_launch(r, p, st, g3_tn_work(p, r, 2.0))) return rc;
+    }
+    if (parts & 2) {
+        const bool direct = pl.nsplit <= 1;
+        if (!direct && (!workspace || workspace_bytes < (size_t)pl.nsplit * Cout * taps * Cin * sizeof(float)))
+            return mpf::fail(MPF_E_SHAPE, "conv_bwd_bf16: workspace too small (mpf_conv_bwd_bf16_workspace_bytes)");
+        G3N p;
+        if (int rc = g3n_fill(p, "conv_bwd_bf16", dy, Cout, 2, x, Cin, 2, static_cast<float*>(workspace), nullptr, rows, Cout, Cin, pl.rps))
+            return rc;
+        if (ksize == 3) {
+            p.Ndim = taps * Cin; p.c_ss = (int64_t)p.Mdim * p.Ndim; p.csb_ss = p.Ndim;
+            p.cv_H = H; p.cv_W = W; p.cv_cin = Cin;
+        }
+        if (direct) { p.c16 = (unsigned short*)dw; p.ldc16 = p.Ndim; }
+        g3n_tiles(p, kBM, 128);
+        const Route r = g3n_route(ksize == 3 ? (const void*)gemm3_nt_kernel<128, true, true> : (const void*)gemm3_nt_kernel<128, true>,
+                                  "conv_bwd_weight_bf16", "mpf_conv_bwd_bf16(weight)", p.ntiles);
+        Work w = g3n_work(p, 2.0, 2.0);
+        if (direct) w.bytes += (2.0 - 4.0) * p.Mdim * p.Ndim;
+        if (int rc = g3_launch(r, p, st, w)) return rc;
+        if (!direct) {
+            const int64_t cn = (int64_t)p.Mdim * p.Ndim;
+            hipLaunchKernelGGL(nt_reduce_kernel<false>, dim3((unsigned)((cn / 2 + 255) / 256)), dim3(256), 0, st, p.c, cn, (const float*)nullptr,
+                               (int64_t)0, p.nsplit, dw, (void*)nullptr);
+            if (int rc = mpf::check(hipGetLastError(), "mpf_conv_bwd_bf16(reduce)")) return rc;
+        }
+    }
+    return parts;
+}
```

Result: faster. 87.65 images/sec, median of 5 (+1.7%).
